# ParBLiSS/kmerhash

Measured on AMD Instinct MI355X. Metric: kmer_inserts_plus_finds_per_sec, higher is better.
Workload: dtype u64

## Files before the change

### kmerhash_amd/csrc/kh_kernels.h

```cpp
#pragma once
#include <hip/hip_runtime.h>
#include <stdint.h>
#include "../../include/kmerhash_amd/kh_hash.h"

#define KH_LB 11
#define KH_L (1u << KH_LB)
#define KH_HS 4096u
#define KH_CHUNK_THREADS 512
#ifndef KH_PART_THREADS
#define KH_PART_THREADS 512
#define KH_PART_MAXPER 4
#endif
#ifndef KH_PART_ITEMS
#define KH_PART_ITEMS 16
#endif
#define KH_PART_TILE (KH_PART_THREADS * KH_PART_ITEMS)
#ifndef KH_PART_STAGE
#define KH_PART_STAGE 4096
#endif
#define KH_NONE 0xFFFFFFFFFFFFFFFFull
#define KH_EMPTY_KEY 0xFFFFFFFFFFFFFFFFull

enum { KHK_RH = 0, KHK_LP = 1 };
enum { KH_FLAG_PROBE_OVERFLOW = 0, KH_FLAG_REGION_OVERFLOW = 1, KH_FLAG_COUNT_OVERFLOW = 2, KH_FLAG_INTERNAL = 3, KH_FLAG_FUSE_INVALID = 4, KH_NFLAGS = 8 };
// ... 406 lines not shown
      for (uint32_t w = 0; w < KH_SCAN_THREADS / 64; ++w) { const uint64_t x = wsum[c][w]; if (w < wid) wpre += x; tot += x; }
      uint64_t ex = running + wpre + incl[c] - ((uint64_t)v[c][0] + v[c][1] + v[c][2] + v[c][3]);
      const uint64_t i0 = base + (uint64_t)c * KH_SCAN_CHUNK + 4 * tid;
#pragma unroll
      for (int j = 0; j < 4; ++j) { if (i0 + j < n) out[i0 + j] = ex; ex += v[c][j]; }
      running += tot;
    }
    __syncthreads();
    if (tid == 0) carry_s = running;
    __syncthreads();
  }
  if (tid == 0) out[n] = carry_s;
}

__global__ __launch_bounds__(256) void k_compact_hits(const uint8_t* __restrict__ flags, const uint64_t* __restrict__ q, const uint32_t* __restrict__ vals,
                               uint64_t n, const uint64_t* __restrict__ tile_off,
                               uint64_t* __restrict__ out_keys, uint32_t* __restrict__ out_vals, uint8_t* __restrict__ out_pairs16) {
  __shared__ uint64_t lk[KH_CMP_TILE];
  __shared__ uint32_t lv[KH_CMP_TILE];
  __shared__ uint32_t wtot[4];
  const uint32_t tid = threadIdx.x, lane = tid & 63, wid = tid >> 6;
  const uint64_t tbase = (uint64_t)blockIdx.x * KH_CMP_TILE;
  const uint64_t base = tbase + (uint64_t)tid * 8;
  uint64_t fw = 0;
  if (base + 8 <= n) fw = *reinterpret_cast<const uint64_t*>(flags + base);
  else for (int j = 0; j < 8; ++j) if (base + j < n && flags[base + j]) fw |= 1ull << (8 * j);
  uint32_t c = 0;
#pragma unroll
  for (int j = 0; j < 8; ++j) c += ((fw >> (8 * j)) & 0xFFu) ? 1u : 0u;
  uint32_t incl = c;
  for (int off = 1; off < 64; off <<= 1) {
    uint32_t o = __shfl_up(incl, off, 64);
    if (lane >= (uint32_t)off) incl += o;
  }
  if (lane == 63) wtot[wid] = incl;
  __syncthreads();
  uint32_t wpre = 0, total = 0;
  for (uint32_t w = 0; w < 4; ++w) { if (w < wid) wpre += wtot[w]; total += wtot[w]; }
  uint32_t x = wpre + incl - c;
#pragma unroll
  for (int j = 0; j < 8; ++j) {
    if ((fw >> (8 * j)) & 0xFFu) { lk[x] = q[base + j]; lv[x] = vals ? vals[base + j] : 0u; ++x; }
  }
  __syncthreads();
  const uint64_t obase = tile_off[blockIdx.x];
  for (uint32_t s = tid; s < total; s += 256) {
    if (out_pairs16) {
      uint4 w;
      w.x = (uint32_t)lk[s]; w.y = (uint32_t)(lk[s] >> 32); w.z = lv[s]; w.w = 0;
      *reinterpret_cast<uint4*>(out_pairs16 + (obase + s) * 16) = w;
    } else {
      out_keys[obase + s] = lk[s];
      if (out_vals) out_vals[obase + s] = lv[s];
    }
  }
}

struct KhTile { uint64_t beg; uint32_t len; uint32_t seg; };
struct KhRec12 { uint32_t klo, khi, val; };

struct KhPartParams {
  const char* kbase; uint32_t kstride;
  const char* vbase; uint32_t vstride;
  uint32_t vconst;
  uint64_t idx_base;
  const ulonglong2* rec_in;
  uint64_t n;
  const KhTile* tiles;
  const uint32_t* ntiles_dev;
  uint32_t ntiles;
  KhSeed seed;
  uint32_t PB;
  uint32_t shift;
  uint32_t nb;
  uint32_t* counts;
  unsigned long long* cursor;
  ulonglong2* orec;
  uint64_t slot;
  uint64_t dump;
  uint32_t* overflow;
  int xcd_swizzle;
  uint64_t slot_in; const unsigned long long* cur_in; uint32_t tps;
  uint64_t sub_slot; uint32_t seg_shift; int xcd_buckets;
};

__device__ __forceinline__ uint32_t kh_part_q(uint64_t h, uint32_t PB) {
  if (PB == 0) return 0;
  uint32_t p = (uint32_t)(h >> KH_LB) & ((1u << PB) - 1u);
  return __brev(p) >> (32 - PB);
}

__device__ __forceinline__ KhTile kh_get_tile(const KhPartParams& P, uint32_t t) {
  if (P.tiles) return P.tiles[t];
  KhTile d;
  d.beg = (uint64_t)t * KH_PART_TILE;
  uint64_t rem = P.n - d.beg;
  d.len = rem < KH_PART_TILE ? (uint32_t)rem : KH_PART_TILE;
  d.seg = 0;
  return d;
}

template <int HASH, bool REC8 = false>
__global__ __launch_bounds__(KH_PART_THREADS) void k_part_hist(KhPartParams P) {
  extern __shared__ __align__(16) uint32_t kh_dyn_smem[];
  uint32_t* hist = kh_dyn_smem;
  const uint32_t tid = threadIdx.x, nb = P.nb;
  const uint32_t ntiles = P.tiles ? *P.ntiles_dev : P.ntiles;
  for (uint32_t i = tid; i < nb; i += KH_PART_THREADS) hist[i] = 0;
  __syncthreads();
  const uint32_t tpb = (ntiles + gridDim.x - 1) / gridDim.x;
  const uint32_t t0 = blockIdx.x * tpb;
  const uint32_t t1 = (t0 + tpb < ntiles) ? t0 + tpb : ntiles;
  uint32_t cur_seg = 0xFFFFFFFFu;
  for (uint32_t t = t0; t < t1; ++t) {
    KhTile d = kh_get_tile(P, t);
    if (d.seg != cur_seg) {
      if (cur_seg != 0xFFFFFFFFu) {
        __syncthreads();
        for (uint32_t i = tid; i < nb; i += KH_PART_THREADS) {
          uint32_t c = hist[i];
          if (c) { atomicAdd(&P.counts[(uint64_t)cur_seg * nb + i], c); hist[i] = 0; }
        }
        __syncthreads();
      }
      cur_seg = d.seg;
    }
    for (uint32_t i = tid; i < d.len; i += KH_PART_THREADS) {
      uint64_t key = P.rec_in ? (REC8 ? reinterpret_cast<const uint64_t*>(P.rec_in)[d.beg + i] : P.rec_in[d.beg + i].x)
                              : *reinterpret_cast<const uint64_t*>(P.kbase + (d.beg + i) * P.kstride);
      uint32_t q = kh_part_q(kh_hash64<HASH>(key, P.seed), P.PB);
      atomicAdd(&hist[(q >> P.shift) & (nb - 1)], 1u);
    }
  }
  __syncthreads();
  if (cur_seg != 0xFFFFFFFFu)
    for (uint32_t i = tid; i < nb; i += KH_PART_THREADS) {
      uint32_t c = hist[i];
      if (c) atomicAdd(&P.counts[(uint64_t)cur_seg * nb + i], c);
    }
}

__device__ __forceinline__ void kh_rec_set(ulonglong2& r, uint64_t key, unsigned long long iv) { r = make_ulonglong2(key, iv); }
__device__ __forceinline__ void kh_rec_set(KhRec12& r, uint64_t key, unsigned long long iv) { r.klo = (uint32_t)key; r.khi = (uint32_t)(key >> 32); r.val = (uint32_t)iv; }
__device__ __forceinline__ void kh_rec_get(const ulonglong2& r, uint64_t& key, unsigned long long& iv) { key = r.x; iv = r.y; }
__device__ __forceinline__ void kh_rec_get(const KhRec12& r, uint64_t& key, unsigned long long& iv) { key = r.klo | ((uint64_t)r.khi << 32); iv = r.val; }
struct KhRec8 { uint64_t key; };
__device__ __forceinline__ void kh_rec_set(KhRec8& r, uint64_t key, unsigned long long) { r.key = key; }
__device__ __forceinline__ void kh_rec_get(const KhRec8& r, uint64_t& key, unsigned long long& iv) { key = r.key; iv = 0; }
template <int RK> struct KhRecOf { typedef ulonglong2 type; };
template <> struct KhRecOf<1> { typedef KhRec12 type; };
template <> struct KhRecOf<2> { typedef KhRec8 type; };
#ifdef KH_PART_OCC3
#define KH_PART_LB(RK) __launch_bounds__(KH_PART_THREADS, (RK) ? 6 : 4)
#define KH_PART_STAGE_OF(RK) ((RK) == 1 ? 3072u : (uint32_t)KH_PART_STAGE)
#else
#define KH_PART_LB(RK) __launch_bounds__(KH_PART_THREADS)
#define KH_PART_STAGE_OF(RK) ((uint32_t)KH_PART_STAGE)
#endif
template <int HASH, int RK>
__global__ KH_PART_LB(RK) void k_part_scatter(KhPartParams P) {
  constexpr bool R12 = RK != 0;
  constexpr uint32_t STAGE = KH_PART_STAGE_OF(RK);
  typedef typename KhRecOf<RK>::type Rec;
  extern __shared__ __align__(16) uint32_t kh_dyn_smem[];
  __shared__ Rec lrec[STAGE];
  __shared__ uint16_t ld[STAGE];
  __shared__ uint32_t wtot[KH_PART_THREADS / 64];
  const uint32_t nb = P.nb;
  uint32_t* hist = kh_dyn_smem;
  uint32_t* loff = kh_dyn_smem + nb;
  unsigned long long* gbase = reinterpret_cast<unsigned long long*>(kh_dyn_smem + 2 * ((nb + 1u) & ~1u));
  const uint32_t tid = threadIdx.x, lane = tid & 63, wid = tid >> 6;
  const uint32_t ntiles = P.tiles ? *P.ntiles_dev : P.ntiles;
  if (blockIdx.x >= ntiles) return;
  uint32_t tile = blockIdx.x;
  const uint32_t xcd = blockIdx.x & 7u;
  if (P.xcd_buckets) {
    const uint32_t j = tile >> 3, per = 8u * P.tps, i = j / per;
    tile = (i * 8u + xcd) * per + (j - i * per);
  } else if (P.xcd_swizzle && (tile | 63u) < ntiles) {
    const uint32_t x = tile & 7u, j = (tile >> 3) & 7u;
    tile = (tile & ~63u) + x * 8u + j;
  }
  KhTile d;
  uint32_t last;
  unsigned long long fill_end = 0;
  if (P.slot_in) {
    const uint32_t seg = tile / P.tps, k = tile - seg * P.tps;
    fill_end = P.cur_in[seg];
    d.seg = seg; d.beg = (uint64_t)seg * P.slot_in + (uint64_t)k * KH_PART_TILE; d.len = 0;
    const uint64_t room = P.slot_in - (uint64_t)k * KH_PART_TILE;
    last = (room < KH_PART_TILE ? (uint32_t)room : KH_PART_TILE) - 1u;
  } else {
    d = kh_get_tile(P, tile);
    if (d.len == 0) return;
    last = d.len - 1u;
  }
  for (uint32_t i = tid; i < nb; i += KH_PART_THREADS) hist[i] = 0;
  uint64_t key[KH_PART_ITEMS];
  unsigned long long iv[KH_PART_ITEMS];
  uint32_t dr[KH_PART_ITEMS];
  if (P.rec_in) {
    const Rec* src = reinterpret_cast<const Rec*>(P.rec_in) + d.beg;
    Rec rr[KH_PART_ITEMS];
#pragma unroll
    for (int j = 0; j < KH_PART_ITEMS; ++j) { const uint32_t i = tid + j * KH_PART_THREADS; rr[j] = src[i < last ? i : last]; }
#pragma unroll
    for (int j = 0; j < KH_PART_ITEMS; ++j) kh_rec_get(rr[j], key[j], iv[j]);
  } else {
    const char* kb = P.kbase + d.beg * P.kstride;
#pragma unroll
    for (int j = 0; j < KH_PART_ITEMS; ++j) {
      const uint32_t i = tid + j * KH_PART_THREADS, ic = i < last ? i : last;
      key[j] = *reinterpret_cast<const uint64_t*>(kb + (uint64_t)ic * P.kstride);
    }
    if (P.vbase) {
      const char* vb = P.vbase + d.beg * P.vstride;
#pragma unroll
      for (int j = 0; j < KH_PART_ITEMS; ++j) {
        const uint32_t i = tid + j * KH_PART_THREADS, ic = i < last ? i : last;
        iv[j] = *reinterpret_cast<const uint32_t*>(vb + (uint64_t)ic * P.vstride);
      }
    } else {
#pragma unroll
      for (int j = 0; j < KH_PART_ITEMS; ++j) iv[j] = P.vconst;
    }
    if (!R12) {
      const uint64_t pos0 = P.idx_base + d.beg;
#pragma unroll
      for (int j = 0; j < KH_PART_ITEMS; ++j) iv[j] |= (unsigned long long)(pos0 + tid + j * KH_PART_THREADS) << 32;
    }
  }
  if (P.slot_in) {
    const uint64_t sbeg = (uint64_t)d.seg * P.slot_in;
    uint64_t fill = fill_end - sbeg;
    if (fill > P.slot_in) fill = P.slot_in;
    const uint64_t off = d.beg - sbeg;
    if (off == (uint64_t)(P.tps - 1u) * KH_PART_TILE && fill > (uint64_t)P.tps * KH_PART_TILE && tid == 0) *P.overflow = 1u;
    d.len = fill > off ? (fill - off < KH_PART_TILE ? (uint32_t)(fill - off) : KH_PART_TILE) : 0u;
    if (d.len == 0) return;
  }
  __syncthreads();
#pragma unroll
  for (int j = 0; j < KH_PART_ITEMS; ++j) {
    const uint32_t i = tid + j * KH_PART_THREADS;
    const uint32_t q = kh_part_q(kh_hash64<HASH>(key[j], P.seed), P.PB);
    const uint32_t dg = (q >> P.shift) & (nb - 1);
    dr[j] = dg << 16;
    if (i < d.len) dr[j] |= atomicAdd(&hist[dg], 1u);
  }
  __syncthreads();
  const uint32_t per = (nb + KH_PART_THREADS - 1) / KH_PART_THREADS;
  uint32_t mine = 0;
  for (uint32_t k = 0; k < per; ++k) { uint32_t b = tid * per + k; if (b < nb) mine += hist[b]; }
  uint32_t incl = mine;
  for (int off = 1; off < 64; off <<= 1) {
    uint32_t o = __shfl_up(incl, off, 64);
// ... 49 lines not shown
      reinterpret_cast<Rec*>(P.orec)[pos] = lrec[s];
    }
  }
}

#define KH_FULLHIST_THREADS 1024
template <int HASH>
__global__ __launch_bounds__(KH_FULLHIST_THREADS) void k_part_hist_full(const char* __restrict__ kbase, uint32_t kstride, uint64_t n, KhSeed seed,
                                                                         uint32_t PB, uint32_t slice, uint32_t slice_bits,
                                                                         uint32_t* __restrict__ counts ) {
  extern __shared__ __align__(16) uint32_t kh_dyn_smem[];
  const uint32_t lb = PB - slice_bits;
  const uint32_t words = lb ? (1u << (lb - 1)) : 1u;
  const uint32_t lmask = (1u << lb) - 1u;
  for (uint32_t i = threadIdx.x; i < words; i += KH_FULLHIST_THREADS) kh_dyn_smem[i] = 0;
  __syncthreads();
  const uint64_t per = (n + gridDim.x - 1) / gridDim.x;
  const uint64_t b0 = (uint64_t)blockIdx.x * per;
  const uint64_t b1 = b0 + per < n ? b0 + per : n;
  for (uint64_t i0 = b0 + threadIdx.x; i0 < b1; i0 += 8 * KH_FULLHIST_THREADS) {
    uint64_t key[8];
#pragma unroll
    for (int j = 0; j < 8; ++j) {
      const uint64_t i = i0 + (uint64_t)j * KH_FULLHIST_THREADS;
      key[j] = i < b1 ? *reinterpret_cast<const uint64_t*>(kbase + i * kstride) : 0ull;
    }
#pragma unroll
    for (int j = 0; j < 8; ++j) {
      if (i0 + (uint64_t)j * KH_FULLHIST_THREADS >= b1) break;
      const uint32_t qg = kh_part_q(kh_hash64<HASH>(key[j], seed), PB);
      if (slice_bits && (qg >> lb) != slice) continue;
      const uint32_t q = qg & lmask;
      const uint32_t sh = 16u * (q & 1u);
      const uint32_t old = atomicAdd(&kh_dyn_smem[q >> 1], 1u << sh);
      if ((((old >> sh) & 0xFFFFu) + 1u) == 0x8000u) {
        atomicSub(&kh_dyn_smem[q >> 1], 0x8000u << sh);
        atomicAdd(&counts[qg], 0x8000u);
      }
    }
  }
  counts += (size_t)slice << lb;
  __syncthreads();
  for (uint32_t i = threadIdx.x; i < words; i += KH_FULLHIST_THREADS) {
    const uint32_t w = kh_dyn_smem[i];
    if (w & 0xFFFFu) atomicAdd(&counts[2 * i], w & 0xFFFFu);
    if (w >> 16) atomicAdd(&counts[2 * i + 1], w >> 16);
  }
}
__global__ void k_seg_offsets(const uint64_t* __restrict__ part_off, uint32_t nb1, uint32_t nb2, uint64_t* __restrict__ segoff,
                              unsigned long long* __restrict__ cur1) {
  const uint32_t s = blockIdx.x * blockDim.x + threadIdx.x;
  if (s <= nb1) { const uint64_t v = part_off[(uint64_t)s * nb2]; segoff[s] = v; if (s < nb1) cur1[s] = v; }
}

__device__ __forceinline__ uint32_t kh_wave_append(bool want, uint32_t* counter);
template <int HASH>
__global__ __launch_bounds__(512) void k_part_direct(const char* __restrict__ kbase, uint32_t kstride, const char* __restrict__ vbase, uint32_t vstride,
                                                     uint32_t vconst, uint64_t n, KhSeed seed, uint32_t PB, ulonglong2* __restrict__ orec,
                                                     unsigned long long* __restrict__ cursor, uint64_t* __restrict__ starts) {
  __shared__ uint32_t cnt;
  const uint32_t q = blockIdx.x, tid = threadIdx.x;
  if (tid == 0) cnt = 0;
  __syncthreads();
  for (uint64_t i0 = 0; i0 < n; i0 += 512) {
    const uint64_t i = i0 + tid;
    bool take = false;
    uint64_t key = 0;
    if (i < n) {
      key = *reinterpret_cast<const uint64_t*>(kbase + i * kstride);
      take = kh_part_q(kh_hash64<HASH>(key, seed), PB) == q;
    }
    const uint32_t pos = kh_wave_append(take, &cnt);
    if (take) {
      const unsigned long long iv = ((unsigned long long)i << 32) | (vbase ? *reinterpret_cast<const uint32_t*>(vbase + i * vstride) : vconst);
      orec[(uint64_t)q * n + pos] = make_ulonglong2(key, iv);
    }
  }
  __syncthreads();
  if (tid == 0) { cursor[q] = (uint64_t)q * n + cnt; starts[q] = (uint64_t)q * n; if (q == 0) starts[gridDim.x] = (uint64_t)gridDim.x * n; }
}

#define KH_SAMPLE_N 65536u
#define KH_SAMPLE_SET (1u << 18)
__global__ void k_sample_dups(const char* __restrict__ kbase, uint32_t kstride, uint64_t n, unsigned long long* __restrict__ set ,
                              uint32_t* __restrict__ dups) {
  const uint32_t i = blockIdx.x * blockDim.x + threadIdx.x;
  if (i >= KH_SAMPLE_N) return;
  const uint64_t pos = (uint64_t)i * (n / KH_SAMPLE_N);
  const unsigned long long key = *reinterpret_cast<const uint64_t*>(kbase + pos * kstride) ^ 0x8000000000000001ull;
  const unsigned long long tag = key ? key : 1ull;
  uint32_t slot = (uint32_t)kh_fmix64(tag) & (KH_SAMPLE_SET - 1);
  for (;;) {
    const unsigned long long cur = atomicCAS(&set[slot], 0ull, tag);
    if (cur == 0ull) break;
    if (cur == tag) { atomicAdd(dups, 1u); break; }
    slot = (slot + 1) & (KH_SAMPLE_SET - 1);
  }
}

__global__ void k_init_cursors2(unsigned long long* __restrict__ cur1, uint64_t n1, uint64_t slot1, uint32_t sub1, unsigned long long* __restrict__ cur2,
                                uint64_t* __restrict__ starts, uint64_t n2, uint64_t slot2, uint32_t* __restrict__ ovf) {
  const uint64_t i = (uint64_t)blockIdx.x * blockDim.x + threadIdx.x;
  if (i < n1 * sub1) cur1[i] = (i / sub1) * slot1 + (i % sub1) * (slot1 / sub1);
  if (i < n2) cur2[i] = i * slot2;
  if (i <= n2) starts[i] = i * slot2;
  if (i == 0) *ovf = 0u;
}
__global__ void k_init_cursors(unsigned long long* __restrict__ cursor, uint64_t* __restrict__ starts, uint64_t n, uint64_t slot) {
  const uint64_t i = (uint64_t)blockIdx.x * blockDim.x + threadIdx.x;
  if (i < n) cursor[i] = i * slot;
  if (starts && i <= n) starts[i] = i * slot;
}

__global__ void k_make_tiles(const uint64_t* __restrict__ segoff, uint32_t nseg, KhTile* __restrict__ tiles, uint32_t* __restrict__ ntiles_out,
                             const unsigned long long* __restrict__ cursor = nullptr, uint64_t slot = 0) {
  __shared__ uint32_t wtot[16];
  __shared__ uint32_t carry_s;
  const uint32_t tid = threadIdx.x, lane = tid & 63, wid = tid >> 6;
  if (tid == 0) carry_s = 0;
  __syncthreads();
  for (uint32_t base = 0; base < nseg; base += 1024) {
    uint32_t s = base + tid;
    uint64_t beg = 0, len = 0;
    if (s < nseg) {
      if (slot) { beg = (uint64_t)s * slot; len = cursor[s] - beg; if (len > slot) len = slot; }
      else { beg = segoff[s]; len = segoff[s + 1] - beg; }
    }
    uint32_t nt = (uint32_t)((len + KH_PART_TILE - 1) / KH_PART_TILE);
    uint32_t incl = nt;
    for (int off = 1; off < 64; off <<= 1) {
      uint32_t o = __shfl_up(incl, off, 64);
      if (lane >= (uint32_t)off) incl += o;
    }
    if (lane == 63) wtot[wid] = incl;
    __syncthreads();
    uint32_t wpre = 0;
    for (uint32_t w = 0; w < wid; ++w) wpre += wtot[w];
    uint32_t carry = carry_s;
    uint32_t first = carry + wpre + incl - nt;
    for (uint32_t k = 0; k < nt; ++k) {
      KhTile d;
      d.beg = beg + (uint64_t)k * KH_PART_TILE;
      uint64_t rem = len - (uint64_t)k * KH_PART_TILE;
      d.len = rem < KH_PART_TILE ? (uint32_t)rem : KH_PART_TILE;
      d.seg = s;
      tiles[first + k] = d;
    }
    __syncthreads();
    if (tid == 1023) carry_s = carry + wpre + incl;
    __syncthreads();
  }
  if (tid == 0) *ntiles_out = carry_s;
}


struct KhMP { long long A; long long n; };
#define KH_MP_NEG (-(1ll << 60))
__device__ __forceinline__ KhMP kh_mp_combine(KhMP first, KhMP then) {
  KhMP r;
  long long a = first.A + then.n;
  r.A = then.A > a ? then.A : a;
  r.n = first.n + then.n;
  return r;
}
__device__ __forceinline__ KhMP kh_block_scan_mp(KhMP v, KhMP* s_wtot, KhMP* total) {
  const uint32_t tid = threadIdx.x, lane = tid & 63, wid = tid >> 6, nw = blockDim.x >> 6;
  KhMP incl = v;
  for (int off = 1; off < 64; off <<= 1) {
    KhMP o;
    o.A = __shfl_up(incl.A, off, 64);
    o.n = __shfl_up(incl.n, off, 64);
    if (lane >= (uint32_t)off) incl = kh_mp_combine(o, incl);
  }
  KhMP excl;
  excl.A = __shfl_up(incl.A, 1, 64);
  excl.n = __shfl_up(incl.n, 1, 64);
  if (lane == 0) { excl.A = KH_MP_NEG; excl.n = 0; }
  __syncthreads();
  if (lane == 63) s_wtot[wid] = incl;
  __syncthreads();
  KhMP wpre; wpre.A = KH_MP_NEG; wpre.n = 0;
  for (uint32_t w = 0; w < wid; ++w) wpre = kh_mp_combine(wpre, s_wtot[w]);
  if (total) {
    KhMP t = wpre;
    for (uint32_t w = wid; w < nw; ++w) t = kh_mp_combine(t, s_wtot[w]);
    *total = t;
  }
  return kh_mp_combine(wpre, excl);
}

// ... 531 lines not shown
      for (uint32_t i = threadIdx.x; i < n; i += KH_CHUNK_THREADS) {
        const uint64_t key = P.ck[b + i];
        f(key, P.cv[b + i], kh_hash64<HASH>(key, P.seed) & mask_n);
      }
    }
  }
}

#define KH_HOMES_PER_THREAD (KH_L / KH_CHUNK_THREADS)

template <int KIND, int HASH>
__global__ __launch_bounds__(KH_CHUNK_THREADS) void k_chunk_count(KhRebuildParams P) {
  __shared__ uint32_t cnt[KH_L];
  __shared__ uint32_t s_emin;
  __shared__ KhMP s_wtot[KH_CHUNK_THREADS / 64];
  const uint32_t tid = threadIdx.x, c = blockIdx.x;
  const uint32_t Ln = P.New.cap > KH_L ? KH_L : (uint32_t)P.New.cap;
  const uint64_t Sc = (uint64_t)c * Ln;
  for (uint32_t i = tid; i < KH_L; i += KH_CHUNK_THREADS) cnt[i] = 0;
  __syncthreads();
  kh_for_each_old<KIND, HASH>(P, c, &s_emin, [&](uint64_t, uint32_t, uint64_t hn) { atomicAdd(&cnt[hn - Sc], 1u); });
  kh_for_each_new<HASH>(P, c, [&](uint64_t, uint32_t, uint64_t hn) { atomicAdd(&cnt[hn - Sc], 1u); });
  __syncthreads();
  KhMP v; v.A = KH_MP_NEG; v.n = 0;
#pragma unroll
  for (uint32_t j = 0; j < KH_HOMES_PER_THREAD; ++j) {
    uint32_t b = tid * KH_HOMES_PER_THREAD + j;
    if (b < Ln) {
      uint32_t cb = cnt[b];
      if (cb > 0xFFFFu) { atomicOr(&P.flags[KH_FLAG_COUNT_OVERFLOW], 1u); cb = 0xFFFFu; }
      P.homecnt[Sc + b] = (uint16_t)cb;
      KhMP h; h.A = (long long)b + cb; h.n = cb;
      v = kh_mp_combine(v, h);
    }
  }
  KhMP total;
  kh_block_scan_mp(v, s_wtot, &total);
  if (tid == 0) { P.sumA[c] = (long long)Sc + total.A; P.sumN[c] = total.n; }
}

#define KH_CARRY_ITEMS 8
__global__ void k_chunk_carry(const long long* __restrict__ sumA, const long long* __restrict__ sumN, uint32_t nch, long long cap,
                              long long* __restrict__ xcarry, KhMP* __restrict__ prefix_tmp) {
  __shared__ KhMP s_wtot[16];
  __shared__ KhMP s_carry;
  const uint32_t tid = threadIdx.x;
  if (tid == 0) { s_carry.A = KH_MP_NEG; s_carry.n = 0; }
  __syncthreads();
  for (uint32_t base = 0; base < nch; base += 1024 * KH_CARRY_ITEMS) {
    const uint32_t c0 = base + tid * KH_CARRY_ITEMS;
    KhMP it[KH_CARRY_ITEMS];
    KhMP v; v.A = KH_MP_NEG; v.n = 0;
#pragma unroll
    for (int j = 0; j < KH_CARRY_ITEMS; ++j) {
      it[j].A = KH_MP_NEG; it[j].n = 0;
      if (c0 + j < nch) { it[j].A = sumA[c0 + j]; it[j].n = sumN[c0 + j]; }
      v = kh_mp_combine(v, it[j]);
    }
    KhMP total;
    KhMP excl = kh_block_scan_mp(v, s_wtot, &total);
    const KhMP carry = s_carry;
    KhMP run = kh_mp_combine(carry, excl);
#pragma unroll
    for (int j = 0; j < KH_CARRY_ITEMS; ++j) {
      if (c0 + j < nch) prefix_tmp[c0 + j] = run;
      run = kh_mp_combine(run, it[j]);
    }
    __syncthreads();
    if (tid == 0) s_carry = kh_mp_combine(carry, total);
    __syncthreads();
  }
  KhMP all = s_carry;
  long long end0 = all.A > all.n ? all.A : all.n;
  long long x0 = end0 - cap;
  if (x0 < 0) x0 = 0;
  for (uint32_t c = tid; c < nch; c += 1024) {
    KhMP p = prefix_tmp[c];
    long long x = x0 + p.n;
    xcarry[c] = p.A > x ? p.A : x;
  }
}

#define KH_SPILL 256
template <int KIND, int HASH>
__global__ __launch_bounds__(KH_CHUNK_THREADS) void k_chunk_place(KhRebuildParams P) {
  __shared__ uint64_t skeys[KH_L + KH_SPILL];
  __shared__ uint32_t svals[KH_L + KH_SPILL];
  __shared__ uint32_t sinfo_w[(KH_L + KH_SPILL) / 4];
  __shared__ uint32_t fill[KH_L];
  __shared__ uint32_t start[KH_L];
  __shared__ uint32_t s_emin;
  __shared__ long long s_pend;
  __shared__ KhMP s_wtot[KH_CHUNK_THREADS / 64];
  uint8_t* sinfo = reinterpret_cast<uint8_t*>(sinfo_w);
  const uint32_t tid = threadIdx.x, c = blockIdx.x;
  const uint32_t Ln = P.New.cap > KH_L ? KH_L : (uint32_t)P.New.cap;
  const uint64_t Sc = (uint64_t)c * Ln, mask_n = P.New.cap - 1;
  const uint32_t empty4 = KIND == KHK_RH ? 0u : 0x40404040u;
  for (uint32_t i = tid; i < KH_L + KH_SPILL; i += KH_CHUNK_THREADS) { skeys[i] = 0; svals[i] = 0; }
  for (uint32_t i = tid; i < (KH_L + KH_SPILL) / 4; i += KH_CHUNK_THREADS) sinfo_w[i] = empty4;
  uint32_t cb[KH_HOMES_PER_THREAD];
  KhMP v; v.A = KH_MP_NEG; v.n = 0;
#pragma unroll
  for (uint32_t j = 0; j < KH_HOMES_PER_THREAD; ++j) {
    uint32_t b = tid * KH_HOMES_PER_THREAD + j;
    cb[j] = b < Ln ? P.homecnt[Sc + b] : 0u;
    if (b < Ln) { KhMP h; h.A = (long long)b + cb[j]; h.n = cb[j]; v = kh_mp_combine(v, h); }
    fill[tid * KH_HOMES_PER_THREAD + j] = 0;
  }
  KhMP excl = kh_block_scan_mp(v, s_wtot, nullptr);
  const long long xr = P.xcarry[c] - (long long)Sc;
  long long p = excl.A > xr + excl.n ? excl.A : xr + excl.n;
#pragma unroll
  for (uint32_t j = 0; j < KH_HOMES_PER_THREAD; ++j) {
    uint32_t b = tid * KH_HOMES_PER_THREAD + j;
    if (b < Ln) {
      long long st = p > (long long)b ? p : (long long)b;
      start[b] = (uint32_t)st;
      p = st + cb[j];
    }
  }
  if (tid == KH_CHUNK_THREADS - 1) s_pend = p;
  __syncthreads();
  auto place = [&](uint64_t key, uint32_t val, uint64_t hn) {
    uint32_t b = (uint32_t)(hn - Sc);
    uint32_t r = atomicAdd(&fill[b], 1u);
    uint32_t prel = start[b] + r;
    uint32_t dist = prel - b;
    uint8_t ib = 0x00;
    if (KIND == KHK_RH) {
      if (dist > 127u) { atomicOr(&P.flags[KH_FLAG_PROBE_OVERFLOW], 1u); dist = 127u; }
      ib = (uint8_t)(0x80u | dist);
    }
    if (prel < KH_L + KH_SPILL) { skeys[prel] = key; svals[prel] = val; sinfo[prel] = ib; }
    else kh_slot_st(P.New.s + ((Sc + prel) & mask_n), key, val, ib);
  };
  kh_for_each_old<KIND, HASH>(P, c, &s_emin, place);
  kh_for_each_new<HASH>(P, c, place);
  __syncthreads();
  long long pend = s_pend;
  if (pend < (long long)Ln) pend = Ln;
  const uint32_t lo = xr > 0 ? (uint32_t)xr : 0u;
  uint32_t hi = pend < (long long)(KH_L + KH_SPILL) ? (uint32_t)pend : (KH_L + KH_SPILL);
  for (uint32_t s0 = lo + tid; s0 < hi; s0 += KH_CHUNK_THREADS) {
    kh_slot_st(P.New.s + ((Sc + s0) & mask_n), skeys[s0], svals[s0], sinfo[s0]);
  }
}

#define KH_XB 127u
#define KH_FSPILL 128u
struct KhFusedParams {
  KhSrcSet src; uint32_t PB;
  KhSlots New; KhSeed seed; int mode;
  unsigned long long* pub;
  uint64_t* ck0; uint32_t* cv0; uint16_t* homecnt0;
  uint32_t* maxidx;
  uint64_t n_total, half_max_load;
  uint64_t base_size;
  unsigned long long* est;
  uint32_t* flags;
  long long poll_limit;
  int nodup;
  KhRebuildParams R;
};

template <int KIND, int HASH, bool MERGE>
__device__ __forceinline__ uint32_t kh_stage_from_table(const KhRebuildParams& R, uint32_t c, uint64_t Sc, unsigned long long* lk,
                                                         unsigned long long* liv, uint32_t* n_staged, uint32_t* scratch) {
  const uint32_t tid = threadIdx.x;
  const uint64_t cap_o = R.Old.cap, mask_o = cap_o - 1, mask_n = R.New.cap - 1;
  if (tid == 0) *n_staged = 0;
  __syncthreads();
  if (cap_o) {
    const uint32_t nch_o = (uint32_t)(cap_o >> KH_LB);
    const uint32_t o = c & (nch_o - 1);
    const bool same = R.New.cap == cap_o;
    const uint64_t S = (uint64_t)o * KH_L;
    uint64_t len = KH_L + 128u;
    if (KIND == KHK_LP) {
      const uint64_t beyond = cap_o - KH_L;
      uint64_t e_total = beyond;
      for (uint64_t base = 0; base < beyond; base += KH_L) {
        const uint32_t window = beyond - base < KH_L ? (uint32_t)(beyond - base) : KH_L;
        __syncthreads();
        if (tid == 0) *scratch = window;
        __syncthreads();
        for (uint32_t t = tid; t < window; t += KH_CHUNK_THREADS) {
          if ((R.Old.s[(S + KH_L + base + t) & mask_o].info & 0xFFu) == 0x40u) { atomicMin(scratch, t); break; }
        }
        __syncthreads();
        const uint32_t e = *scratch;
        e_total = base + e;
        if (e < window) break;
      }
      __syncthreads();
      if (tid == 0) *scratch = 0;
      len = KH_L + e_total;
    }
    if (KIND == KHK_RH) {
      constexpr uint32_t NS = (KH_L + 128u + KH_CHUNK_THREADS - 1) / KH_CHUNK_THREADS;
      uint4 w[NS];
#pragma unroll
      for (uint32_t it = 0; it < NS; ++it) {
        const uint32_t t = it * KH_CHUNK_THREADS + tid;
        w[it] = kh_slot_ld(R.Old.s + ((S + (t < KH_L + 128u ? t : KH_L + 127u)) & mask_o));
      }
#pragma unroll
      for (uint32_t it = 0; it < NS; ++it) {
        const uint64_t sl = (S + it * KH_CHUNK_THREADS + tid) & mask_o;
        const uint32_t inf = it * KH_CHUNK_THREADS + tid < KH_L + 128u ? (w[it].w & 0xFFu) : 0u;
        bool take = false;
        uint32_t hrel = 0;
        const uint64_t key = kh_slot_key(w[it]);
        if (inf >= 0x80u && !(R.drop_marked && (w[it].w & KH_INFO_ERASE_MARK))) {
          const uint64_t home_o = (sl - (inf & 0x7Fu)) & mask_o;
          if ((uint32_t)(home_o >> KH_LB) == o) {
            if (same) { take = true; hrel = (uint32_t)(home_o - S); }
            else {
              const uint64_t hn = kh_hash64<HASH>(key, R.seed) & mask_n;
              take = (uint32_t)(hn >> KH_LB) == c;
              hrel = (uint32_t)(hn - Sc);
            }
          }
        }
        const uint32_t x = kh_wave_append(take, n_staged);
        if (take && x < KH_DD_M) { lk[x] = key; liv[x] = MERGE ? (unsigned long long)w[it].z : (((unsigned long long)hrel << 32) | w[it].z); }
      }
    } else
    for (uint64_t t0 = 0; t0 < len; t0 += KH_CHUNK_THREADS) {
      const uint64_t t = t0 + tid;
      bool take = false;
      uint64_t key = 0; uint32_t val = 0, hrel = 0;
      if (t < len) {
        const uint4 w = kh_slot_ld(R.Old.s + ((S + t) & mask_o));
        if ((w.w & 0xFFu) < 0x40u) {
          key = kh_slot_key(w);
          const uint64_t h = kh_hash64<HASH>(key, R.seed);
          if ((uint32_t)((h & mask_o) >> KH_LB) == o && (uint32_t)((h & mask_n) >> KH_LB) == c) {
            take = true; val = w.z; hrel = (uint32_t)((h & mask_n) - Sc);
          }
        }
      }
      const uint32_t x = kh_wave_append(take, n_staged);
      if (take && x < KH_DD_M) { lk[x] = key; liv[x] = MERGE ? (unsigned long long)val : (((unsigned long long)hrel << 32) | val); }
    }
  }
  if (!MERGE)
    kh_for_each_new<HASH>(R, c, [&](uint64_t key, uint32_t val, uint64_t hn) {
      const uint32_t x = kh_wave_append(true, n_staged);
      if (x < KH_DD_M) { lk[x] = key; liv[x] = ((unsigned long long)(uint32_t)(hn - Sc) << 32) | val; }
    });
  __syncthreads();
  return *n_staged;
}

#ifdef KH_TRACE
__device__ unsigned long long kh_trace[512 * 12];
#ifndef KH_TRACE_SRC
#define KH_TRACE_SRC 0
#endif
#define KH_STAMP(i) do { if (SRC == KH_TRACE_SRC && threadIdx.x == 0 && blockIdx.x >= 20000 && blockIdx.x < 20512) kh_trace[(blockIdx.x - 20000) * 12 + (i)] = clock64(); } while (0)
#else
#define KH_STAMP(i)
#endif
template <int KIND, int HASH, int SRC>
__global__ __launch_bounds__(KH_CHUNK_THREADS) void k_build_fused(KhFusedParams P) {
  __shared__ unsigned long long lk[KH_DD_M];
  __shared__ unsigned long long liv[KH_DD_M];
  __shared__ uint32_t set[KH_HS];
  __shared__ __align__(8) uint16_t simg[KH_L + KH_FSPILL];
  __shared__ KhMP32 s_wtot[KH_CHUNK_THREADS / 64];
  __shared__ uint32_t s_chunk, s_x, s_max, s_abort;
  __shared__ long long s_pend;
  static_assert(KH_HS >= 2 * KH_L, "set[] is reused as cnt/fill + start");
  uint32_t* cnt = set;
  uint32_t* start = set + KH_L;
  const uint32_t tid = threadIdx.x;
  const uint64_t cap = P.New.cap, mask_n = cap - 1;
  const uint32_t nch = (uint32_t)(cap >> KH_LB);
  KH_STAMP(0);
  if (tid == 0) {
    s_chunk = blockIdx.x;
    s_max = 0;
    s_abort = (SRC == 0 || SRC == 2) ? (uint32_t)__hip_atomic_load(&P.est[1], __ATOMIC_RELAXED, __HIP_MEMORY_SCOPE_AGENT) : 0u;
  }
  __syncthreads();
  const ulonglong2** s_ptr = reinterpret_cast<const ulonglong2**>(simg);
  uint32_t* s_cum = reinterpret_cast<uint32_t*>(simg) + 2 * KH_MAX_SRC;
  static_assert((KH_L + KH_FSPILL) * 2 >= KH_MAX_SRC * 8 + (KH_MAX_SRC + 1) * 4, "source table fits the image array");
  const uint32_t c = s_chunk;
  const uint64_t Sc = (uint64_t)c * KH_L;
  const unsigned long long VALID = 1ull << 63;
  uint32_t m, rep_mask;
  uint32_t vote_old = 0, vote_rec = 0;
  if (SRC == 0) {
    const uint32_t q = P.PB ? (__brev(c) >> (32 - P.PB)) : 0u;
    const KhSrcView V = kh_src_setup<true>(P.src, q, s_ptr, s_cum);
    m = V.m;
    KH_STAMP(1);
    vote_rec = m;
    const bool aborted = s_abort != 0;
    if (m >= KH_DD_M || aborted) {
      if (tid == 0) {
        if (!aborted) atomicOr(&P.flags[KH_FLAG_FUSE_INVALID], 1u);
        __hip_atomic_store(&P.pub[c], VALID, __ATOMIC_RELAXED, __HIP_MEMORY_SCOPE_AGENT);
      }
      return;
    }
    const bool nodup = P.nodup && c != 0;
    if (!nodup) for (uint32_t s = tid; s < KH_HS; s += KH_CHUNK_THREADS) set[s] = 0;
    if (m) {
      ulonglong2 rr[KH_DD_M / KH_CHUNK_THREADS];
      const uint32_t last = m - 1u;
      if (V.one12) {
        KhRec12 r3[KH_DD_M / KH_CHUNK_THREADS];
#pragma unroll
        for (uint32_t it = 0; it < KH_DD_M / KH_CHUNK_THREADS; ++it) { const uint32_t i = it * KH_CHUNK_THREADS + tid; r3[it] = V.one12[i < last ? i : last]; }
#pragma unroll
        for (uint32_t it = 0; it < KH_DD_M / KH_CHUNK_THREADS; ++it) rr[it] = make_ulonglong2(r3[it].klo | ((uint64_t)r3[it].khi << 32), (unsigned long long)r3[it].val);
      } else if (V.one) {
#pragma unroll
        for (uint32_t it = 0; it < KH_DD_M / KH_CHUNK_THREADS; ++it) { const uint32_t i = it * KH_CHUNK_THREADS + tid; rr[it] = V.one[i < last ? i : last]; }
      } else {
        const ulonglong2* pp[KH_DD_M / KH_CHUNK_THREADS];
#pragma unroll
        for (uint32_t it = 0; it < KH_DD_M / KH_CHUNK_THREADS; ++it) { const uint32_t i = it * KH_CHUNK_THREADS + tid; pp[it] = kh_src_addr(V, s_ptr, s_cum, i < last ? i : last); }
#pragma unroll
        for (uint32_t it = 0; it < KH_DD_M / KH_CHUNK_THREADS; ++it) rr[it] = *pp[it];
      }
#pragma unroll
      for (uint32_t it = 0; it < KH_DD_M / KH_CHUNK_THREADS; ++it) {
        const uint32_t i = it * KH_CHUNK_THREADS + tid;
        if (i < m) { lk[i] = rr[it].x; liv[i] = rr[it].y; }
      }
    }
    if (V.n > 1) __syncthreads();
    for (uint32_t i = tid; i < KH_L + KH_FSPILL; i += KH_CHUNK_THREADS) simg[i] = 0xFFFFu;
    __syncthreads();
    if (nodup) {
      rep_mask = 0;
#pragma unroll
      for (uint32_t it = 0; it < KH_DD_M / KH_CHUNK_THREADS; ++it) if (it * KH_CHUNK_THREADS + tid < m) rep_mask |= 1u << it;
    } else rep_mask = kh_dd_fold(lk, liv, set, m, P.mode, P.seed.xk);
    __syncthreads();
    KH_STAMP(2);
  } else if (SRC == 2) {
    const uint32_t q = P.PB ? (__brev(c) >> (32 - P.PB)) : 0u;
    const KhSrcView V = kh_src_setup(P.src, q, s_ptr, s_cum);
    for (uint32_t s = tid; s < KH_HS; s += KH_CHUNK_THREADS) set[s] = 0;
    if (s_abort != 0) {
      if (tid == 0) __hip_atomic_store(&P.pub[c], VALID, __ATOMIC_RELAXED, __HIP_MEMORY_SCOPE_AGENT);
      return;
    }
    const uint32_t n_old = kh_stage_from_table<KIND, HASH, true>(P.R, c, Sc, lk, liv, &s_x, &s_max);
    KH_STAMP(1);
    m = n_old + V.m;
    vote_old = n_old; vote_rec = V.m;
    if (n_old >= KH_DD_M || m >= KH_DD_M) {
      if (tid == 0) {
        atomicOr(&P.flags[KH_FLAG_FUSE_INVALID], 1u);
        __hip_atomic_store(&P.pub[c], VALID, __ATOMIC_RELAXED, __HIP_MEMORY_SCOPE_AGENT);
      }
      return;
// ... 234 lines not shown
    constexpr uint32_t KH_DUPK = 3;
    uint32_t ei[KH_DD_M / KH_CHUNK_THREADS][KH_DUPK];
#pragma unroll
    for (uint32_t it = 0; it < KH_DD_M / KH_CHUNK_THREADS; ++it)
#pragma unroll
      for (uint32_t d = 0; d < KH_DUPK; ++d) ei[it][d] = simg[pr[it] + d < gend[it] ? pr[it] + d : 0u] & 0x7FFu;
    bool more = false;
#pragma unroll
    for (uint32_t it = 0; it < KH_DD_M / KH_CHUNK_THREADS; ++it) {
#pragma unroll
      for (uint32_t d = 0; d < KH_DUPK; ++d)
        if (kh_keq(lk[ei[it][d]], mykey[it], P.seed.xk) && pr[it] + d < gend[it]) dup = true;
      pr[it] += KH_DUPK;
      more = more || pr[it] < gend[it];
    }
    while (__any(more)) {
      more = false;
#pragma unroll
      for (uint32_t it = 0; it < KH_DD_M / KH_CHUNK_THREADS; ++it) {
        if (pr[it] < gend[it]) {
          if (kh_keq(lk[simg[pr[it]] & 0x7FFu], mykey[it], P.seed.xk)) dup = true;
          ++pr[it];
          more = more || pr[it] < gend[it];
        }
      }
    }
    if (__any(dup) && (tid & 63) == 0) atomicOr(&P.flags[KH_FLAG_FUSE_INVALID], 1u);
  }
  KH_STAMP(7);
  long long pend = s_pend;
  if (pend < (long long)KH_L) pend = KH_L;
  const uint32_t lo = (uint32_t)xr;
  const uint32_t hi = pend < (long long)(KH_L + KH_FSPILL) ? (uint32_t)pend : (KH_L + KH_FSPILL);
  for (uint32_t s0 = lo + tid; s0 < hi; s0 += KH_CHUNK_THREADS) {
    KhSlot* dst = P.New.s + ((Sc + s0) & mask_n);
    const uint32_t e = simg[s0];
    if (e == 0xFFFFu) kh_slot_st(dst, 0, 0, kh_empty_info<KIND>());
    else {
      const uint32_t x = e & 0x7FFu;
      const uint64_t key = lk[x];
      uint32_t ib = 0x00u;
      if (KIND == KHK_RH) {
        uint32_t dist = e >> 11;
        if (dist == 31u) {
          dist = s0 - (uint32_t)((kh_hash64<HASH>(key, P.seed) & mask_n) - Sc);
          if (dist > 127u) dist = 127u;
        }
        ib = 0x80u | dist;
      }
      kh_slot_st(dst, key, (uint32_t)liv[x], ib);
    }
  }
  KH_STAMP(8);
}

#ifdef KH_TRACE
#define KH_STAMP_L(i) do { if (threadIdx.x == 0 && blockIdx.x >= 20000 && blockIdx.x < 20512) kh_trace[(blockIdx.x - 20000) * 12 + (i)] = clock64(); } while (0)
#else
#define KH_STAMP_L(i)
#endif
#define KH_LEAN_M 2016u
template <int KIND, int HASH>
__global__ __launch_bounds__(KH_CHUNK_THREADS, 8) void k_build_lean(KhFusedParams P) {
  __shared__ unsigned long long lk[KH_LEAN_M];
  __shared__ uint32_t lv[KH_LEAN_M];
  __shared__ __align__(16) uint32_t cnt16[KH_L / 2];
  __shared__ __align__(8) uint16_t start0[KH_L];
  __shared__ __align__(16) uint16_t u_sort[KH_L + KH_LEAN_M];
  uint16_t* npre = u_sort;
  uint16_t* sidx = u_sort + KH_L;
  uint16_t* simg = u_sort;
  static_assert(KH_L + KH_LEAN_M >= KH_L + KH_FSPILL, "the slot image fits over the sort arrays");
  static_assert(((KH_L + KH_FSPILL) * 2) % 16 == 0 && (KH_L * 2) % 16 == 0, "filled with 16-byte stores");
  __shared__ KhMP32 s_wtot[KH_CHUNK_THREADS / 64];
  __shared__ uint32_t s_x, s_abort;
  __shared__ long long s_pend;
  const uint32_t tid = threadIdx.x;
  const uint64_t cap = P.New.cap, mask_n = cap - 1;
  const uint32_t nch = (uint32_t)(cap >> KH_LB);
  const uint32_t c = blockIdx.x;
  const uint64_t Sc = (uint64_t)c * KH_L;
  const unsigned long long VALID = 1ull << 63;
  KH_STAMP_L(0);
  if (tid == 0) s_abort = (uint32_t)__hip_atomic_load(&P.est[1], __ATOMIC_RELAXED, __HIP_MEMORY_SCOPE_AGENT);
  const uint32_t q = P.PB ? (__brev(c) >> (32 - P.PB)) : 0u;
  const KhRec12* src; uint32_t m;
  KhRec12 r3[KH_DD_M / KH_CHUNK_THREADS];
  unsigned long long kreg[KH_DD_M / KH_CHUNK_THREADS];
  if (P.src.slot[0]) {
    const uint64_t b = (uint64_t)q * P.src.slot[0];
    src = reinterpret_cast<const KhRec12*>(P.src.rec[0]) + b;
    const uint32_t last = (uint32_t)P.src.slot[0] - 1u;
#pragma unroll
    for (uint32_t it = 0; it < KH_DD_M / KH_CHUNK_THREADS; ++it) { const uint32_t i = it * KH_CHUNK_THREADS + tid; r3[it] = src[i < last ? i : last]; }
    const uint64_t e = P.src.cur[0][q] - b;
    m = (uint32_t)(e < P.src.slot[0] ? e : P.src.slot[0]);
  } else {
    const uint64_t b = P.src.off[0][q];
    src = reinterpret_cast<const KhRec12*>(P.src.rec[0]) + b;
    m = (uint32_t)(P.src.off[0][q + 1] - b);
    const uint32_t last = m ? m - 1u : 0u;
    const KhRec12* from = m ? src : reinterpret_cast<const KhRec12*>(P.src.rec[0]);
#pragma unroll
    for (uint32_t it = 0; it < KH_DD_M / KH_CHUNK_THREADS; ++it) { const uint32_t i = it * KH_CHUNK_THREADS + tid; r3[it] = from[i < last ? i : last]; }
  }
  kh_lds_fill16(cnt16, sizeof(cnt16), 0u);
  __syncthreads();
  const bool aborted = s_abort != 0;
  if (m >= KH_LEAN_M || aborted) {
    if (tid == 0) {
      if (!aborted) atomicOr(&P.flags[KH_FLAG_FUSE_INVALID], 1u);
      __hip_atomic_store(&P.pub[c], VALID, __ATOMIC_RELAXED, __HIP_MEMORY_SCOPE_AGENT);
    }
    return;
  }
  uint32_t hb[KH_DD_M / KH_CHUNK_THREADS];
#pragma unroll
  for (uint32_t it = 0; it < KH_DD_M / KH_CHUNK_THREADS; ++it) {
    const uint32_t i = it * KH_CHUNK_THREADS + tid;
    kreg[it] = r3[it].klo | ((uint64_t)r3[it].khi << 32);
    hb[it] = 0;
    if (i < m) {
      lk[i] = kreg[it]; lv[i] = r3[it].val;
      hb[it] = (uint32_t)((kh_hash64<HASH>(kreg[it], P.seed) & mask_n) - Sc) & (KH_L - 1u);
      atomicAdd(&cnt16[hb[it] >> 1], 1u << (16 * (hb[it] & 1)));
    }
  }
  KH_STAMP_L(1);
  __syncthreads();
  KH_STAMP_L(2);
  uint32_t cb[KH_HOMES_PER_THREAD];
  KhMP32 v; v.A = KH_MP32_NEG; v.n = 0;
#pragma unroll
  for (uint32_t j = 0; j < KH_HOMES_PER_THREAD; ++j) {
    const uint32_t b = tid * KH_HOMES_PER_THREAD + j;
    cb[j] = (cnt16[b >> 1] >> (16 * (b & 1))) & 0xFFFFu;
    KhMP32 h; h.A = (int)(b + cb[j]); h.n = (int)cb[j];
    v = kh_mp_combine(v, h);
  }
  KhMP32 total;
  const KhMP32 excl = kh_block_scan_mp32(v, s_wtot, &total);
  const uint32_t n_c = (uint32_t)total.n;
  const long long spill0 = total.A > (long long)KH_L ? total.A - (long long)KH_L : 0;
  const bool early = n_c + KH_XB <= KH_L;
  KH_STAMP_L(3);
  if (c == 0) {
    bool dup = false;
#pragma unroll
    for (uint32_t it = 0; it < KH_DD_M / KH_CHUNK_THREADS; ++it) {
      const uint32_t x = it * KH_CHUNK_THREADS + tid;
      if (x < m) {
        for (uint32_t y = x + 1; y < m; ++y) dup = dup || kh_keq(lk[y], kreg[it], P.seed.xk);
      }
    }
    if (__any(dup) && (tid & 63) == 0) atomicOr(&P.flags[KH_FLAG_FUSE_INVALID], 1u);
    if (tid == 0) {
      if (!early) atomicOr(&P.flags[KH_FLAG_FUSE_INVALID], 1u);
      __hip_atomic_store(&P.pub[0], VALID | ((unsigned long long)spill0 << 32) | n_c, __ATOMIC_RELAXED, __HIP_MEMORY_SCOPE_AGENT);
      P.maxidx[0] = 0;
    }
#pragma unroll
    for (uint32_t j = 0; j < KH_HOMES_PER_THREAD; ++j) P.homecnt0[tid * KH_HOMES_PER_THREAD + j] = (uint16_t)cb[j];
    for (uint32_t x = tid; x < m; x += KH_CHUNK_THREADS) { P.ck0[x] = lk[x]; P.cv0[x] = lv[x]; }
    return;
  }
  unsigned long long w0 = 0;
  if (tid == 0) {
    if (c < 64) {
      const unsigned long long mine = ((unsigned long long)n_c << 32) | m;
      const unsigned long long tot = atomicAdd(&P.est[0], mine) + mine;
      const uint32_t sn = (uint32_t)(tot >> 32), sm = (uint32_t)tot;
      if ((c == 63 || (nch < 64 && c == nch - 1)) && sm > 0) {
        const double dhat = (double)P.base_size + (double)P.n_total * (double)sn / (double)sm * 1.15;
        if (dhat <= (double)P.half_max_load) {
          atomicOr(&P.flags[KH_FLAG_FUSE_INVALID], 1u);
          __hip_atomic_store(&P.est[1], 1ull, __ATOMIC_RELAXED, __HIP_MEMORY_SCOPE_AGENT);
        }
      }
    }
    if (early) __hip_atomic_store(&P.pub[c], VALID | ((unsigned long long)spill0 << 32) | n_c, __ATOMIC_RELAXED, __HIP_MEMORY_SCOPE_AGENT);
    w0 = __hip_atomic_load(&P.pub[c - 1], __ATOMIC_RELAXED, __HIP_MEMORY_SCOPE_AGENT);
    P.maxidx[c] = 0;
  }
  {
    long long p = excl.A > (long long)excl.n ? excl.A : excl.n;
    uint32_t np = (uint32_t)excl.n;
    uint32_t st4[KH_HOMES_PER_THREAD], np4[KH_HOMES_PER_THREAD];
#pragma unroll
    for (uint32_t j = 0; j < KH_HOMES_PER_THREAD; ++j) {
      const uint32_t b = tid * KH_HOMES_PER_THREAD + j;
      const long long st = p > (long long)b ? p : (long long)b;
      st4[j] = (uint32_t)st & 0xFFFFu;
      np4[j] = np;
      p = st + cb[j];
      np += cb[j];
    }
    static_assert(KH_HOMES_PER_THREAD == 4, "two packed counter words, one 8-byte store of starts / counts per thread");
    reinterpret_cast<uint2*>(start0)[tid] = make_uint2(st4[0] | (st4[1] << 16), st4[2] | (st4[3] << 16));
    reinterpret_cast<uint2*>(npre)[tid] = make_uint2(np4[0] | (np4[1] << 16), np4[2] | (np4[3] << 16));
    if (tid == KH_CHUNK_THREADS - 1) s_pend = p;
    cnt16[tid * (KH_HOMES_PER_THREAD / 2)] = 0; cnt16[tid * (KH_HOMES_PER_THREAD / 2) + 1] = 0;
  }
  __syncthreads();
  uint32_t pj[KH_DD_M / KH_CHUNK_THREADS];
#pragma unroll
  for (uint32_t it = 0; it < KH_DD_M / KH_CHUNK_THREADS; ++it) {
    pj[it] = 0;
    const uint32_t x = it * KH_CHUNK_THREADS + tid;
    if (x < m) {
      const uint32_t b = hb[it];
      const uint32_t r = (atomicAdd(&cnt16[b >> 1], 1u << (16 * (b & 1))) >> (16 * (b & 1))) & 0xFFFFu;
      uint32_t j = npre[b] + r;
      if (j >= KH_LEAN_M) j = KH_LEAN_M - 1u;
      sidx[j] = (uint16_t)x;
      pj[it] = (start0[b] + r) | (j << 16);
    }
  }
  __syncthreads();
  KH_STAMP_L(4);
  {
    bool dup = false;
    uint32_t jn[KH_DD_M / KH_CHUNK_THREADS], gend[KH_DD_M / KH_CHUNK_THREADS];
#pragma unroll
    for (uint32_t it = 0; it < KH_DD_M / KH_CHUNK_THREADS; ++it) {
      gend[it] = 0;
      const uint32_t x = it * KH_CHUNK_THREADS + tid;
      if (x < m) {
        const uint32_t b = hb[it];
        gend[it] = npre[b] + ((cnt16[b >> 1] >> (16 * (b & 1))) & 0xFFFFu);
        if (gend[it] > KH_LEAN_M) gend[it] = KH_LEAN_M;
      }
      jn[it] = (pj[it] >> 16) + 1u;
    }
    constexpr uint32_t KH_DUPK = 3;
    uint32_t ei[KH_DD_M / KH_CHUNK_THREADS][KH_DUPK];
#pragma unroll
    for (uint32_t it = 0; it < KH_DD_M / KH_CHUNK_THREADS; ++it)
#pragma unroll
      for (uint32_t d = 0; d < KH_DUPK; ++d) ei[it][d] = sidx[jn[it] + d < gend[it] ? jn[it] + d : 0u];
    bool more = false;
#pragma unroll
    for (uint32_t it = 0; it < KH_DD_M / KH_CHUNK_THREADS; ++it) {
#pragma unroll
      for (uint32_t d = 0; d < KH_DUPK; ++d)
        if (kh_keq(lk[ei[it][d] < KH_LEAN_M ? ei[it][d] : 0u], kreg[it], P.seed.xk) && jn[it] + d < gend[it]) dup = true;
      jn[it] += KH_DUPK;
      more = more || jn[it] < gend[it];
    }
    while (__any(more)) {
      more = false;
#pragma unroll
      for (uint32_t it = 0; it < KH_DD_M / KH_CHUNK_THREADS; ++it) {
        if (jn[it] < gend[it]) {
          const uint32_t e = sidx[jn[it]];
          if (kh_keq(lk[e < KH_LEAN_M ? e : 0u], kreg[it], P.seed.xk)) dup = true;
          ++jn[it];
          more = more || jn[it] < gend[it];
        }
      }
    }
    if (__any(dup) && (tid & 63) == 0) atomicOr(&P.flags[KH_FLAG_FUSE_INVALID], 1u);
  }
  KH_STAMP_L(5);
  if (tid == 0) {
    unsigned long long w = w0;
// ... 502 lines not shown
    uint32_t dist = pos - b;
    if (dist > 127u) { atomicOr(&P.flags[KH_FLAG_PROBE_OVERFLOW], 1u); dist = 127u; }
    if (pos < KH_L + KH_FSPILL) { ikey[pos] = key; ival[pos] = val; iinfo[pos] = (uint8_t)(0x80u | dist); }
    else kh_slot_st(P.New.s + ((Sc + pos) & mask_n), key, val, 0x80u | dist);
  };
  uint32_t late = 0;
  uint32_t pj[ROWS + 2];
#pragma unroll
  for (uint32_t k = 0; k < ROWS; ++k) {
    pj[k] = 0;
    if ((keep >> k) & 1u) {
      const uint32_t b = rank[k] >> 16, r = rank[k] & 0xFFFFu;
      const uint32_t p0 = start0[b] + r, j = npre[b] + r;
      pj[k] = (p0 & 0xFFFFu) | (j << 16);
      if (p0 >= KH_XB + j) enter(kh_slot_key(w[k]), w[k].z, b, p0); else late |= 1u << k;
    }
  }
#pragma unroll
  for (uint32_t u = 0; u < 2; ++u) {
    pj[ROWS + u] = 0;
    if (rrank[u] != 0xFFFFFFFFu) {
      const uint32_t i = tid + u * KH_CHUNK_THREADS;
      const uint32_t b = hbr[u], r = rrank[u];
      const uint32_t p0 = start0[b] + r, j = npre[b] + r;
      pj[ROWS + u] = (p0 & 0xFFFFu) | (j << 16);
      if (p0 >= KH_XB + j) enter(rk[i], (uint32_t)riv[i], b, p0); else late |= 1u << (ROWS + u);
    }
  }
  if (tid == 0) {
    unsigned long long ww = w0;
    const long long t0 = clock64();
    while (!(ww & VALID)) {
      if (clock64() - t0 > P.poll_limit) { atomicOr(&P.flags[KH_FLAG_FUSE_INVALID], 1u); ww = VALID; break; }
      __builtin_amdgcn_s_sleep(4);
      ww = __hip_atomic_load(&P.pub[c - 1], __ATOMIC_RELAXED, __HIP_MEMORY_SCOPE_AGENT);
    }
    const uint32_t x = (uint32_t)((ww >> 32) & 0x7FFFFFFFu);
    if (x > KH_XB) atomicOr(&P.flags[KH_FLAG_FUSE_INVALID], 1u);
    if (!early) {
      const long long e = (long long)x + n_c;
      const long long pe = (long long)total.A > e ? (long long)total.A : e;
      const long long sp = pe > (long long)KH_L ? pe - (long long)KH_L : 0;
      __hip_atomic_store(&P.pub[c], VALID | ((unsigned long long)sp << 32) | n_c, __ATOMIC_RELAXED, __HIP_MEMORY_SCOPE_AGENT);
    }
    s_x = x > KH_XB ? 0u : x;
  }
  __syncthreads();
  const uint32_t xr = s_x;
#pragma unroll
  for (uint32_t k = 0; k < ROWS; ++k) {
    if ((late >> k) & 1u) {
      const uint32_t p0 = pj[k] & 0xFFFFu, pc = (pj[k] >> 16) + xr;
      enter(kh_slot_key(w[k]), w[k].z, rank[k] >> 16, p0 > pc ? p0 : pc);
    }
  }
#pragma unroll
  for (uint32_t u = 0; u < 2; ++u) {
    if ((late >> (ROWS + u)) & 1u) {
      const uint32_t i = tid + u * KH_CHUNK_THREADS;
      const uint32_t p0 = pj[ROWS + u] & 0xFFFFu, pc = (pj[ROWS + u] >> 16) + xr;
      enter(rk[i], (uint32_t)riv[i], hbr[u], p0 > pc ? p0 : pc);
    }
  }
  __syncthreads();
  {
    const int tA = total.A > 0 ? total.A : 0;
    int pend = tA > (int)xr + (int)n_c ? tA : (int)xr + (int)n_c;
    if (pend < (int)KH_L) pend = (int)KH_L;
    if (pend > (int)(KH_L + KH_FSPILL)) pend = (int)(KH_L + KH_FSPILL);
#pragma unroll
    for (uint32_t k = 0; k < ROWS; ++k) {
      const int s0 = (int)(base + 64u * k);
      if (k < nrows && s0 >= (int)xr && s0 < pend) {
        const uint32_t ib = iinfo[s0];
        KhSlot* dst = P.New.s + ((Sc + (uint32_t)s0) & mask_n);
        if (ib == 0u) kh_slot_st(dst, 0, 0, kh_empty_info<KHK_RH>());
        else kh_slot_st(dst, ikey[s0], ival[s0], ib);
      }
    }
  }
  (void)n_old;
}

__global__ void k_fused_tail_carry(const unsigned long long* __restrict__ pub, uint32_t nch, long long* __restrict__ xcarry0,
                                   uint64_t* __restrict__ noff0 = nullptr, uint32_t* __restrict__ ncnt0 = nullptr) {
  if (threadIdx.x == 0 && blockIdx.x == 0) {
    xcarry0[0] = (long long)((pub[nch - 1] >> 32) & 0x7FFFFFFFull);
    if (noff0) { noff0[0] = 0; noff0[1] = 0; }
    if (ncnt0) ncnt0[0] = (uint32_t)pub[0];
  }
}

__global__ __launch_bounds__(1024) void k_fused_totals(const unsigned long long* __restrict__ pub, const uint32_t* __restrict__ maxidx, uint32_t nch,
                                                       unsigned long long* __restrict__ totals) {
  __shared__ unsigned long long ws[16];
  __shared__ uint32_t wm[16];
  unsigned long long sum = 0; uint32_t mx = 0;
  for (uint32_t c = blockIdx.x * 1024 + threadIdx.x; c < nch; c += gridDim.x * 1024) { sum += pub[c] & 0xFFFFFFFFull; const uint32_t v = maxidx[c]; mx = v > mx ? v : mx; }
  for (int off = 32; off > 0; off >>= 1) { sum += __shfl_down(sum, off, 64); const uint32_t o = __shfl_down(mx, off, 64); mx = o > mx ? o : mx; }
  if ((threadIdx.x & 63) == 0) { ws[threadIdx.x >> 6] = sum; wm[threadIdx.x >> 6] = mx; }
  __syncthreads();
  if (threadIdx.x == 0) {
    unsigned long long t = 0; uint32_t m = 0;
    for (int w = 0; w < 16; ++w) { t += ws[w]; m = wm[w] > m ? wm[w] : m; }
    if (t) atomicAdd(&totals[0], t);
    if (m) atomicMax(&totals[1], (unsigned long long)m);
  }
}

__global__ void k_disp_hist(const KhSlot* __restrict__ slots, uint64_t cap, unsigned long long* __restrict__ out128) {
  __shared__ uint32_t h[128];
  if (threadIdx.x < 128) h[threadIdx.x] = 0;
  __syncthreads();
  uint64_t i = (uint64_t)blockIdx.x * blockDim.x + threadIdx.x;
  uint64_t stride = (uint64_t)gridDim.x * blockDim.x;
  for (; i < cap; i += stride) { uint32_t b = slots[i].info & 0xFFu; if (b >= 0x80u) atomicAdd(&h[b & 0x7Fu], 1u); }
  __syncthreads();
  if (threadIdx.x < 128 && h[threadIdx.x]) atomicAdd(&out128[threadIdx.x], (unsigned long long)h[threadIdx.x]);
}

template <int KIND>
__global__ void k_unpack_slots(const KhSlot* __restrict__ slots, uint64_t cap, uint64_t* __restrict__ keys, uint32_t* __restrict__ vals,
                               uint8_t* __restrict__ info, uint8_t* __restrict__ flags) {
  uint64_t i = (uint64_t)blockIdx.x * blockDim.x + threadIdx.x;
  uint64_t stride = (uint64_t)gridDim.x * blockDim.x;
  for (; i < cap; i += stride) {
    const uint4 w = kh_slot_ld(slots + i);
    if (keys) keys[i] = kh_slot_key(w);
    if (vals) vals[i] = w.z;
    if (info) info[i] = (uint8_t)(w.w & 0xFFu);
    if (flags) flags[i] = kh_is_occupied<KIND>(w.w & 0xFFu) ? 1 : 0;
  }
}

#define KH_SHARD_THREADS 512
#define KH_SHARD_TILE(KW) (KH_SHARD_THREADS * KhKey<KW>::SHARD_ITEMS)
#define KH_SHARD_MAXR 64
struct KhShardAdj { long long a[8]; __host__ __device__ KhShardAdj() { for (int i = 0; i < 8; ++i) a[i] = 0; } };
__global__ void k_shard_piece_bounds(const uint64_t* __restrict__ tile_off, uint32_t ntiles, uint32_t p, uint32_t pieces, uint64_t* __restrict__ out ) {
  const uint32_t j = blockIdx.x * blockDim.x + threadIdx.x;
  if (j >= p * (pieces + 1)) return;
  const uint32_t r = j / (pieces + 1), i = j % (pieces + 1);
  out[j] = tile_off[(uint64_t)r * ntiles + (uint64_t)ntiles * i / pieces];
}
template <int HASH, int KW>
__device__ __forceinline__ uint32_t kh_rank_of(typename KhKey<KW>::key_t key, typename KhKey<KW>::seed_t seed, uint32_t p, uint32_t pmask) {
  const uint64_t h = KhKey<KW>::template hash<HASH>(key, seed);
  return pmask ? (uint32_t)(h & pmask) : (uint32_t)(h % p);
}
template <int HASH, int KW>
__global__ __launch_bounds__(KH_SHARD_THREADS) void k_shard_count(const uint64_t* __restrict__ keys, uint64_t n, typename KhKey<KW>::seed_t seed, uint32_t p,
                                                                  uint32_t pmask, uint32_t* __restrict__ tile_counts , uint32_t ntiles) {
  typedef KhKey<KW> K;
  __shared__ uint32_t h[KH_SHARD_MAXR];
  if (threadIdx.x < KH_SHARD_MAXR) h[threadIdx.x] = 0;
  __syncthreads();
  const uint64_t base = (uint64_t)blockIdx.x * KH_SHARD_TILE(KW);
  typename K::key_t key[K::SHARD_ITEMS];
#pragma unroll
  for (uint32_t k = 0; k < K::SHARD_ITEMS; ++k) {
    const uint64_t i = base + threadIdx.x + k * KH_SHARD_THREADS;
    key[k] = K::load(keys, i < n ? i : n - 1);
  }
  if (p <= 8) {
    unsigned long long c0 = 0, c1 = 0;
#pragma unroll
    for (uint32_t k = 0; k < K::SHARD_ITEMS; ++k) {
      const uint64_t i = base + threadIdx.x + k * KH_SHARD_THREADS;
      if (i < n) {
        const uint32_t r = kh_rank_of<HASH, KW>(key[k], seed, p, pmask);
        if (r < 4) c0 += 1ull << (16 * r); else c1 += 1ull << (16 * (r - 4));
      }
    }
// ... 640 lines not shown
```

### kmerhash_amd/csrc/kmerhash_amd.hip

```cpp
#include "kh_kernels.h"
#include "kh_kernels_wide.h"
#include "kh_kernels_values.h"
#include "kh_kernels_index.h"
#include "kh_kernels_index_wide.h"
#include "kh_kernels_csr.h"
#include "kh_kernels_chain.h"
#include "kh_kernels_edits.h"
#include "kh_kernels_cigar.h"
#include "kh_kernels_ends.h"
#include "kh_part_sizing.h"
#include "kh_scratch.h"
#include "../../include/kmerhash_amd.h"

#include <string>
#include <vector>
#include <cstdio>
#include <cstring>
#include <algorithm>
#include <cmath>
#include <cstdlib>

#include <map>
#include <memory>
#include <mutex>
// ... 44 lines not shown
    e = hipMalloc(&p, bytes);
    if (e != hipSuccess) return e;
  }
  std::lock_guard<std::mutex> g(P.m);
  P.size_of[p] = bytes;
  *out = p;
  return hipSuccess;
}
void pool_free(int dev, void* p) {
  if (!p) return;
  DevPool& P = g_pool[dev & 15];
  {
    std::lock_guard<std::mutex> g(P.m);
    auto it = P.size_of.find(p);
    if (it != P.size_of.end()) {
      P.free_.insert(std::make_pair(it->second, p));
      P.cached += it->second;
      return;
    }
  }
  hipFree(p);
}
struct HostPool { std::mutex m; std::vector<uint64_t*> pinned; std::vector<hipEvent_t> events[16]; };
HostPool g_host;
uint64_t* pinned_get() {
  { std::lock_guard<std::mutex> g(g_host.m);
    if (!g_host.pinned.empty()) { uint64_t* p = g_host.pinned.back(); g_host.pinned.pop_back(); return p; } }
  uint64_t* p = nullptr;
  if (hipHostMalloc(reinterpret_cast<void**>(&p), 64 * sizeof(uint64_t)) != hipSuccess) { (void)hipGetLastError(); return nullptr; }
  return p;
}
void pinned_put(uint64_t* p) { if (p) { std::lock_guard<std::mutex> g(g_host.m); g_host.pinned.push_back(p); } }
hipEvent_t event_get(int dev) {
  { std::lock_guard<std::mutex> g(g_host.m);
    auto& v = g_host.events[dev & 15];
    if (!v.empty()) { hipEvent_t e = v.back(); v.pop_back(); return e; } }
  hipEvent_t e = nullptr;
  hipEventCreate(&e);
  return e;
}
void event_put(int dev, hipEvent_t e) { if (e) { std::lock_guard<std::mutex> g(g_host.m); g_host.events[dev & 15].push_back(e); } }
}

namespace {

struct ProfRec { const char* name; hipEvent_t a, b; };

struct Block { char* p; size_t cap; };

}

struct SlackShared { unsigned long long* cur2; uint64_t* starts; uint32_t* ovf; uint64_t slot; };
struct SlotBuf {
  void* p; uint64_t cap;
  SlotBuf() : p(nullptr), cap(0) {}
  SlotBuf(KhSlots s) : p(s.s), cap(s.cap) {}
  SlotBuf(KwSlots s) : p(s.s), cap(s.cap) {}
};
struct kh_table {
  int kind = KHK_RH, hash = 0, device = 0;
  KhSeed seed = KhSeed{0, 0u};
  hipStream_t stream = nullptr;
  float min_lf = 0.f, max_lf = 0.f;
  uint64_t min_load = 0, max_load = 0, lsize = 0;
  uint32_t slot_bytes = sizeof(KhSlot);
  SlotBuf cur, spare;
  std::vector<Block> blocks;
  size_t blk = 0, off = 0;
  uint64_t* hpin = nullptr;
  std::string err;
  struct {
    bool active, fallback, nodup; int mode;
    bool repeatable, slack, rec12;
    SlackShared sh;
    uint64_t n_total, fed, cap_u; uint32_t PB;
    ulonglong2 *tmp, *fin;
    KhSrcSet S;
    uint64_t* stage_k; uint32_t* stage_v;
    const uint64_t* wk[KH_MAX_SRC]; const uint32_t* wv[KH_MAX_SRC]; uint64_t wn[KH_MAX_SRC]; uint32_t wsrc; uint32_t* wcnt;
  } ins = {};
  uint32_t* part_overflow = nullptr;
  double batch_vf = 1.0;
  bool batch_nodup = false;
  bool prof = false;
  std::vector<ProfRec> recs;
  std::vector<std::pair<std::string, std::pair<double, uint64_t> > > prof_acc;
};
struct kh_wtable : kh_table {};

namespace {

inline uint64_t next_pow2(uint64_t x) {
  if (x <= 1) return 1;
  return uint64_t(1) << (64 - __builtin_clzll(x - 1));
}
inline uint64_t threshold(uint64_t buckets, float lf) {
  return static_cast<uint64_t>(static_cast<float>(buckets) * lf);
}
inline uint32_t log2u(uint64_t x) { return 63u - (uint32_t)__builtin_clzll(x); }

kh_status fail(kh_table* t, kh_status s, const std::string& msg) {
  if (t) t->err = msg;
  return s;
}
inline kh_status hip_status(hipError_t e) { return e == hipSuccess ? KH_OK : e == hipErrorOutOfMemory ? KH_ERR_NOMEM : KH_ERR_HIP; }
kh_status hip_fail(kh_table* t, const char* call, hipError_t e) {
  if (t) t->err = std::string(call) + ": " + hipGetErrorString(e);
  return hip_status(e);
}
#define HIPCHK_T(table, call)                                                                          \
  do {                                                                                                 \
    hipError_t e__ = (call);                                                                           \
    if (e__ != hipSuccess) return hip_fail(table, #call, e__);                                         \
  } while (0)
#define HIPCHK(call) HIPCHK_T(t, call)
#define HIPCHK0(call) HIPCHK_T(nullptr, call)

inline int cu_count(int device) {
  int ncu = 256;
  hipDeviceGetAttribute(&ncu, hipDeviceAttributeMultiprocessorCount, device);
  return ncu > 0 ? ncu : 256;
}
inline int cu_count(const kh_table* t) { return cu_count(t->device); }

class Scratch {
 public:
  Scratch(int device, hipStream_t stream) : device_(device), stream_(stream) {}
  Scratch(const Scratch&) = delete;
  Scratch& operator=(const Scratch&) = delete;
  ~Scratch() { finish(); }

  hipError_t error() const { return err_; }
  bool ok() const { return err_ == hipSuccess; }
  void check(hipError_t e) { if (err_ == hipSuccess) err_ = e; }
  bool launched() { check(hipGetLastError()); busy_ = true; return ok(); }

  void* alloc(size_t bytes) {
    void* p = nullptr;
    if (ok() && nblk_ == kMaxBlocks) err_ = hipErrorInvalidValue;
    if (ok()) err_ = pool_alloc(device_, bytes, &p);
    if (!ok()) return nullptr;
    blk_[nblk_++] = p;
    busy_ = true;
    return p;
  }
  template <typename F> size_t measure(F&& layout) { car_ = KhCarver(); layout(*this); return car_.size(); }
  template <typename F> void carve(void* base, F&& layout) { car_ = KhCarver(base); layout(*this); }
  template <typename F> bool layout(F&& layout) {
    const size_t bytes = measure(layout);
    void* p = bytes ? alloc(bytes) : nullptr;
    if (bytes && !p) return false;
    carve(p, layout);
    return ok();
  }
  template <typename T> T* take(uint64_t count) { return car_.take<T>(count); }
  template <typename T> const T* in(const T* p, uint64_t count, kh_mem where) {
    if (where != KH_MEM_HOST) return p;
    T* d = car_.take<T>(count);
    if (d) copy(d, p, count * sizeof(T), hipMemcpyHostToDevice);
    return d;
  }
  template <typename T> T* out(T* p, uint64_t count, kh_mem where) {
    if (where != KH_MEM_HOST) return p;
    T* d = car_.take<T>(count);
    if (d && nout_ == kMaxOut) check(hipErrorInvalidValue);
    else if (d) outs_[nout_++] = Out{p, d};
// ... 135 lines not shown
    if (st != KH_OK) return st;
  }
  s = Slots{static_cast<decltype(s.s)>(b.p), cap};
  if (g_poison) {
    if (is_wide(t)) hipLaunchKernelGGL(kw_poison, slots_grid(cap), dim3(256), 0, t->stream, wide(b));
    else hipLaunchKernelGGL(k_poison, slots_grid(cap), dim3(256), 0, t->stream, narrow(b));
    HIPCHK(hipGetLastError());
  }
  return KH_OK;
}
void retire_slots(kh_table* t, SlotBuf s) {
  if (!s.p) return;
  if (t->spare.p) { hipStreamSynchronize(t->stream); free_slots(t, t->spare); }
  t->spare = s;
}
void adopt_slots(kh_table* t, SlotBuf nw) {
  const SlotBuf old = t->cur;
  t->cur = nw;
  retire_slots(t, old);
  t->min_load = threshold(nw.cap, t->min_lf);
  t->max_load = threshold(nw.cap, t->max_lf);
}

struct Launch {
  kh_table* t; const char* name; hipEvent_t a, b; bool on;
  Launch(kh_table* t_, const char* n) : t(t_), name(n), a(nullptr), b(nullptr), on(t_ && t_->prof) {
    if (on) { a = event_get(t->device); b = event_get(t->device); hipEventRecord(a, t->stream); }
  }
  ~Launch() {
    if (on) { hipEventRecord(b, t->stream); ProfRec r; r.name = name; r.a = a; r.b = b; t->recs.push_back(r); }
  }
};
void prof_collect(kh_table* t) {
  if (t->recs.empty()) return;
  hipStreamSynchronize(t->stream);
  for (auto& r : t->recs) {
    float ms = 0.f;
    hipEventElapsedTime(&ms, r.a, r.b);
    event_put(t->device, r.a); event_put(t->device, r.b);
    bool found = false;
    for (auto& a : t->prof_acc) if (a.first == r.name) { a.second.first += ms; a.second.second += 1; found = true; break; }
    if (!found) t->prof_acc.push_back(std::make_pair(std::string(r.name), std::make_pair(double(ms), uint64_t(1))));
  }
  t->recs.clear();
}

#define KH_SWITCH_HASH(h, ...)                                                        \
  switch (h) {                                                                        \
    case KHH_IDENTITY: { constexpr int HASH = KHH_IDENTITY; __VA_ARGS__; } break;     \
    case KHH_MURMUR3_X86: { constexpr int HASH = KHH_MURMUR3_X86; __VA_ARGS__; } break; \
    case KHH_MURMUR3_X64: { constexpr int HASH = KHH_MURMUR3_X64; __VA_ARGS__; } break; \
    default: { constexpr int HASH = KHH_FARM; __VA_ARGS__; } break;                   \
  }
#define KH_SWITCH_KIND_HASH(k, h, ...)                                                \
  if ((k) == KHK_RH) { constexpr int KIND = KHK_RH; KH_SWITCH_HASH(h, __VA_ARGS__) }  \
  else { constexpr int KIND = KHK_LP; KH_SWITCH_HASH(h, __VA_ARGS__) }

inline uint32_t grid_for(uint64_t n, uint32_t block, uint32_t maxblocks = 256 * 16) {
  uint64_t g = (n + block - 1) / block;
  if (g < 1) g = 1;
  if (g > maxblocks) g = maxblocks;
  return (uint32_t)g;
}

template <typename T>
kh_status stage_in(kh_table* t, const void* p, uint64_t n, kh_mem where, const T** out) {
  if (where == KH_MEM_DEVICE || p == nullptr) { *out = static_cast<const T*>(p); return KH_OK; }
  T* d = nullptr;
  TAKE(d, T, n);
  HIPCHK(hipMemcpyAsync(d, p, sizeof(T) * n, hipMemcpyHostToDevice, t->stream));
  *out = d;
  return KH_OK;
}

inline size_t ws_rebuild(uint64_t cap) { return size_t(cap) * 2 + (cap > KH_L ? (cap >> KH_LB) : 1) * 48 + (size_t(1) << 16); }

struct PreCount { uint16_t* homecnt; long long* sumA; long long* sumN; };

const bool g_disable_fused_rebuild = getenv("KH_DISABLE_FUSED_BUILD") != nullptr || getenv("KH_DISABLE_FUSED_REBUILD") != nullptr;

const long long g_poll_limit = getenv("KH_DEBUG_POLL_LIMIT") ? atoll(getenv("KH_DEBUG_POLL_LIMIT")) : (1ll << 23);
struct FusedRun { unsigned long long* totals; uint32_t* flags; };
const bool g_disable_lean = getenv("KH_DISABLE_LEAN_BUILD") != nullptr;
kh_status launch_fused(kh_table* t, int src, KhFusedParams& F, const KhSlots& nw, uint32_t PB_tail, const char* name, FusedRun* out) {
  const uint32_t nch = (uint32_t)(nw.cap >> KH_LB);
  char* blk; uint32_t* maxidx; uint64_t* ck0; uint32_t* cv0; uint16_t* hc0; long long* xc0; uint64_t* noff0; uint32_t* ncnt0;
  const size_t sz_pub = (size_t)nch * 8, sz_ctl = sz_pub + 256, sz_all = sz_ctl + (size_t)nch * 4;
  TAKE(blk, char, sz_all);
  maxidx = reinterpret_cast<uint32_t*>(blk + sz_ctl);
  TAKE(ck0, uint64_t, KH_DD_M); TAKE(cv0, uint32_t, KH_DD_M); TAKE(hc0, uint16_t, KH_L); TAKE(xc0, long long, 1);
  TAKE(noff0, uint64_t, 2); TAKE(ncnt0, uint32_t, 1);
  HIPCHK(hipMemsetAsync(blk, 0, sz_all, t->stream));
  F.New = nw; F.seed = t->seed;
  F.pub = reinterpret_cast<unsigned long long*>(blk);
  unsigned long long* totals = reinterpret_cast<unsigned long long*>(blk + sz_pub);
  F.maxidx = maxidx; F.ck0 = ck0; F.cv0 = cv0; F.homecnt0 = hc0;
  F.est = reinterpret_cast<unsigned long long*>(blk + sz_pub + 32);
  F.flags = reinterpret_cast<uint32_t*>(blk + sz_pub + 64);
  F.poll_limit = g_poll_limit;
  F.R.New = nw; F.R.seed = t->seed; F.R.flags = F.flags;
  { Launch L(t, name);
    const double mean_c = (double)F.n_total / (double)nch;
    const bool lean_fits = mean_c + 5.0 * std::sqrt(mean_c) < (double)KH_LEAN_M;
    if (src == 0 && F.nodup && F.src.rec12 == 1 && F.src.n == 1 && lean_fits && !g_disable_lean) { KH_SWITCH_KIND_HASH(t->kind, t->hash, hipLaunchKernelGGL((k_build_lean<KIND, HASH>), dim3(nch), dim3(KH_CHUNK_THREADS), 0, t->stream, F)); }
    else if (src == 0) { KH_SWITCH_KIND_HASH(t->kind, t->hash, hipLaunchKernelGGL((k_build_fused<KIND, HASH, 0>), dim3(nch), dim3(KH_CHUNK_THREADS), 0, t->stream, F)); }
    else if (src == 1) { KH_SWITCH_KIND_HASH(t->kind, t->hash, hipLaunchKernelGGL((k_build_fused<KIND, HASH, 1>), dim3(nch), dim3(KH_CHUNK_THREADS), 0, t->stream, F)); }
    else if (src == 3) { KH_SWITCH_HASH(t->hash, hipLaunchKernelGGL((k_build_fused<KHK_RH, HASH, 3>), dim3(nch), dim3(KH_CHUNK_THREADS), 0, t->stream, F)); }
    else if (src == 4) { KH_SWITCH_HASH(t->hash, hipLaunchKernelGGL((k_erase_stream<HASH>), dim3(nch), dim3(KH_CHUNK_THREADS), 0, t->stream, F)); }
    else if (src == 5) { KH_SWITCH_HASH(t->hash, hipLaunchKernelGGL((k_insert_stream<HASH>), dim3(nch), dim3(KH_CHUNK_THREADS), 0, t->stream, F)); }
    else { KH_SWITCH_KIND_HASH(t->kind, t->hash, hipLaunchKernelGGL((k_build_fused<KIND, HASH, 2>), dim3(nch), dim3(KH_CHUNK_THREADS), 0, t->stream, F)); } }
  { Launch L(t, "k_fused_totals");
    hipLaunchKernelGGL(k_fused_totals, dim3(std::max<uint32_t>(1u, std::min<uint32_t>(64u, nch / 1024u))), dim3(1024), 0, t->stream, F.pub, maxidx, nch, totals); }
  {
    Launch L(t, "k_fused_tail");
    hipLaunchKernelGGL(k_fused_tail_carry, dim3(1), dim3(64), 0, t->stream, F.pub, nch, xc0, noff0, ncnt0);
    KhRebuildParams T0;
    memset(&T0, 0, sizeof(T0));
    T0.Old = kNoSlots; T0.New = nw; T0.ck = ck0; T0.cv = cv0; T0.noff = noff0; T0.ncnt = ncnt0; T0.PB = PB_tail;
    T0.seed = t->seed; T0.homecnt = hc0; T0.xcarry = xc0; T0.flags = F.flags;
    KH_SWITCH_KIND_HASH(t->kind, t->hash, hipLaunchKernelGGL((k_chunk_place<KIND, HASH>), dim3(1), dim3(KH_CHUNK_THREADS), 0, t->stream, T0));
  }
  HIPCHK(hipGetLastError());
  HIPCHK(hipMemcpyAsync(t->hpin, blk + sz_pub, 128, hipMemcpyDeviceToHost, t->stream));
  t->hpin[30] = 0;
  if (t->part_overflow) HIPCHK(hipMemcpyAsync(t->hpin + 30, t->part_overflow, 4, hipMemcpyDeviceToHost, t->stream));
  HIPCHK(hipStreamSynchronize(t->stream));
  out->totals = totals; out->flags = F.flags;
  return KH_OK;
}

const char* const kProbeOverflowText = "Robin Hood probe distance would exceed 127 (7-bit info field, hashmap_robinhood.hpp:142-144,556)";
const char* const kDedupOverflowText = "internal: de-duplication set overflow";
kh_status flags_status(kh_table* t, const uint32_t* f) {
  if (f[KH_FLAG_PROBE_OVERFLOW]) return fail(t, KH_ERR_PROBE_OVERFLOW, kProbeOverflowText);
  if (f[KH_FLAG_REGION_OVERFLOW]) return fail(t, KH_ERR_PROBE_OVERFLOW, "cluster longer than one chunk (2048 slots) without an empty slot");
  if (f[KH_FLAG_COUNT_OVERFLOW]) return fail(t, KH_ERR_PROBE_OVERFLOW, "more than 65535 keys share one home bucket");
  if (f[KH_FLAG_INTERNAL]) return fail(t, KH_ERR_HIP, kDedupOverflowText);
  return KH_OK;
}

struct Narrow {
  typedef KhSlots Slots; typedef KhRebuildParams Params;
  static Slots view(const SlotBuf& b) { return narrow(b); }
  static void set_seed(Params& P, const kh_table* t) { P.seed = t->seed; }
  static void count(kh_table* t, uint32_t nch, const Params& P) {
    Launch L(t, "k_chunk_count");
    KH_SWITCH_KIND_HASH(t->kind, t->hash, hipLaunchKernelGGL((k_chunk_count<KIND, HASH>), dim3(nch), dim3(KH_CHUNK_THREADS), 0, t->stream, P));
  }
  static void place(kh_table* t, uint32_t nch, const Params& P) {
    Launch L(t, "k_chunk_place");
    KH_SWITCH_KIND_HASH(t->kind, t->hash, hipLaunchKernelGGL((k_chunk_place<KIND, HASH>), dim3(nch), dim3(KH_CHUNK_THREADS), 0, t->stream, P));
  }
};
struct Wide {
  typedef KwSlots Slots; typedef KwRebuildParams Params;
  static Slots view(const SlotBuf& b) { return wide(b); }
  static void set_seed(Params& P, const kh_table* t) { P.seed = t->seed.s; }
  static void count(kh_table* t, uint32_t nch, const Params& P) {
    Launch L(t, "kw_chunk_count");
    KH_SWITCH_HASH(t->hash, hipLaunchKernelGGL((kw_chunk_count<HASH>), dim3(nch), dim3(KW_DD_THREADS), 0, t->stream, P));
  }
  static void place(kh_table* t, uint32_t nch, const Params& P) {
    Launch L(t, "kw_chunk_place");
    KH_SWITCH_HASH(t->hash, hipLaunchKernelGGL((kw_chunk_place<HASH>), dim3(nch), dim3(KW_DD_THREADS), 0, t->stream, P));
  }
};
template <typename W>
kh_status relayout(kh_table* t, typename W::Slots nw, const uint64_t* ck, const uint32_t* cv, const uint64_t* noff, const uint32_t* ncnt,
                   uint32_t PB, bool drop_marked, const PreCount* pre) {
  const uint32_t nch = nw.cap > KH_L ? (uint32_t)(nw.cap >> KH_LB) : 1u;
  uint16_t* homecnt; long long *sumA, *sumN, *xcarry; KhMP* ptmp; uint32_t* flags;
  if (pre) { homecnt = pre->homecnt; sumA = pre->sumA; sumN = pre->sumN; }
  else { TAKE(homecnt, uint16_t, nw.cap); TAKE(sumA, long long, nch); TAKE(sumN, long long, nch); }
  TAKE(xcarry, long long, nch);
  TAKE(ptmp, KhMP, nch);
  TAKE(flags, uint32_t, KH_NFLAGS);
  HIPCHK(hipMemsetAsync(flags, 0, sizeof(uint32_t) * KH_NFLAGS, t->stream));
  typename W::Params P;
  memset(&P, 0, sizeof(P));
  P.Old = W::view(t->cur); P.drop_marked = drop_marked ? 1 : 0; P.New = nw; P.ck = ck; P.cv = cv; P.noff = noff; P.ncnt = ncnt; P.PB = PB;
  if (t->lsize == 0) P.Old.cap = 0;
  W::set_seed(P, t); P.homecnt = homecnt; P.sumA = sumA; P.sumN = sumN; P.xcarry = xcarry; P.flags = flags;
  if (!pre) W::count(t, nch, P);
  { Launch L(t, "k_chunk_carry");
    hipLaunchKernelGGL(k_chunk_carry, dim3(1), dim3(1024), 0, t->stream, sumA, sumN, nch, (long long)nw.cap, xcarry, ptmp); }
  W::place(t, nch, P);
  HIPCHK(hipGetLastError());
  HIPCHK(hipMemcpyAsync(t->hpin, flags, sizeof(uint32_t) * KH_NFLAGS, hipMemcpyDeviceToHost, t->stream));
  HIPCHK(hipStreamSynchronize(t->stream));
  const kh_status st = flags_status(t, reinterpret_cast<const uint32_t*>(t->hpin));
  if (st != KH_OK) { retire_slots(t, nw); return st; }
  adopt_slots(t, nw);
  return KH_OK;
}

kh_status rebuild(kh_table* t, uint64_t new_cap, const uint64_t* ck, const uint32_t* cv, const uint64_t* noff,
                  const uint32_t* ncnt, uint32_t PB, bool drop_marked, uint64_t total_after, const PreCount* pre = nullptr) {
  if (total_after > new_cap)
    return fail(t, KH_ERR_FULL, "table would hold more elements than buckets (no slot to insert into)");
  if (is_wide(t)) {
    KwSlots nw;
    kh_status st = fresh_slots(t, new_cap, nw);
    return st != KH_OK ? st : relayout<Wide>(t, nw, ck, cv, noff, ncnt, PB, drop_marked, nullptr);
  }
  KhSlots nw;
  kh_status st = fresh_slots(t, new_cap, nw);
  if (st != KH_OK) return st;
  const bool from_empty = t->lsize == 0;
  if (!pre && !g_disable_fused_rebuild && new_cap >= 2 * (uint64_t)KH_L && total_after <= threshold(new_cap, 0.9f) &&
      (!noff || PB >= log2u(new_cap >> KH_LB)) &&
      (from_empty ? noff != nullptr
                  : (t->cur.cap >= 2 * (uint64_t)KH_L && (new_cap == t->cur.cap || new_cap == 2 * t->cur.cap)))) {
    const size_t keep_blk = t->blk, keep_off = t->off;
    KhFusedParams F;
    memset(&F, 0, sizeof(F));
    F.PB = PB; F.mode = KH_DEDUP_FIRST;
    F.R.Old = narrow(t->cur); F.R.drop_marked = drop_marked ? 1 : 0; F.R.ck = ck; F.R.cv = cv; F.R.noff = noff; F.R.ncnt = ncnt; F.R.PB = PB;
    if (from_empty) F.R.Old.cap = 0;
    FusedRun run;
    { kh_status fs = launch_fused(t, 1, F, nw, log2u(new_cap >> KH_LB), "k_rebuild_fused", &run); if (fs != KH_OK) return fs; }
    const uint32_t* ff = reinterpret_cast<const uint32_t*>(reinterpret_cast<const char*>(t->hpin) + 64);
    bool bad = false;
    for (int i = 0; i < KH_NFLAGS; ++i) bad = bad || ff[i] != 0;
    if (!bad && t->hpin[0] == total_after) {
      adopt_slots(t, nw);
      return KH_OK;
    }
    if (getenv("KH_DEBUG_FUSED"))
      fprintf(stderr, "[kmerhash_amd] fused rebuild rejected: placed %llu expected %llu flags=%u %u %u %u %u\n", (unsigned long long)t->hpin[0],
              (unsigned long long)total_after, ff[0], ff[1], ff[2], ff[3], ff[4]);
    if (ff[KH_FLAG_PROBE_OVERFLOW] && !ff[KH_FLAG_FUSE_INVALID]) {
      retire_slots(t, nw);
      return fail(t, KH_ERR_PROBE_OVERFLOW, kProbeOverflowText);
    }
    t->blk = keep_blk; t->off = keep_off;
  }
  return relayout<Narrow>(t, nw, ck, cv, noff, ncnt, PB, drop_marked, pre);
}

inline uint64_t rh_rehash_capacity(uint64_t c, uint64_t size, float max_lf) {
  if (size > 0) {
    if (0 >= threshold(c, max_lf)) c <<= 1;
    while (size > threshold(c, max_lf)) c <<= 1;
  }
  return c;
}
kh_status refuse_streaming(kh_table* t) { return fail(t, KH_ERR_INVALID, "a streamed insert is in progress (kh_insert_end first)"); }
kh_status do_rehash(kh_table* t, uint64_t b) {
  if (t->ins.active) return refuse_streaming(t);
  uint64_t n = next_pow2(b);
  if (n == t->cur.cap) return KH_OK;
  if (t->kind == KHK_RH) {
    n = rh_rehash_capacity(n, t->lsize, t->max_lf);
    if (n == t->cur.cap) return KH_OK;
  } else if (t->lsize > n) {
    return fail(t, KH_ERR_FULL, "ERROR: did not find any place to insert.  should not have happend (hashmap_linearprobe.hpp:408)");
  }
  { kh_status ps = arena_prepare(t, ws_rebuild(n)); if (ps != KH_OK) return ps; }
  return rebuild(t, n, nullptr, nullptr, nullptr, nullptr, 0, false, t->lsize);
}
kh_status do_reserve(kh_table* t, uint64_t n) {
  if (n > t->max_load) return do_rehash(t, static_cast<uint64_t>(static_cast<float>(n) / t->max_lf));
  return KH_OK;
}

struct Partitioned {
  ulonglong2* rec;
  uint64_t* part_off;
  uint32_t PB, nparts;
  ulonglong2* spare;
  uint64_t slot;
  const unsigned long long* cursor;
  uint32_t* overflow;
  int rec12;
};
const bool g_disable_slack = getenv("KH_DISABLE_SLACK_PARTITION") != nullptr;
const int g_xcd_swizzle = getenv("KH_DISABLE_XCD_SWIZZLE") ? 0 : 1;
const int g_xcd_fronts = getenv("KH_DISABLE_XCD_FRONTS") ? 0 : 1;
inline uint32_t xcd_fronts_min_tiles() { const char* e = getenv("KH_XCD_FRONTS_MIN_TILES"); return e ? (uint32_t)std::max(0, atoi(e)) : 4u; }
inline uint64_t part_buffer_records(uint64_t n, uint32_t PB, bool allow_slack, double vf = 1.0) {
  if (!allow_slack || g_disable_slack || PB <= 11 || n < (uint64_t(256) << PB)) return n;
  return (slack_slot((double)n / (double)(uint64_t(1) << PB), vf) << PB) + KH_PART_TILE;
}

kh_status partition_batch(kh_table* t, const char* kbase, uint32_t kstride, const char* vbase, uint32_t vstride,
                          uint32_t vconst, uint64_t n, uint64_t idx_base, uint32_t PB, ulonglong2* tmp, ulonglong2* fin, Partitioned& out,
                          bool allow_slack = false, int rec12 = 0, const SlackShared* shared = nullptr, bool force_slack = false, double vf = 1.0) {
  const uint32_t nparts = 1u << PB;
  out.slot = 0; out.cursor = nullptr; out.overflow = nullptr; out.rec12 = 0;
  if (shared || force_slack || part_buffer_records(n, PB, allow_slack, vf) != n) {
    const uint32_t B1 = (PB + 1) / 2, B2 = PB - B1, nb1 = 1u << B1, nb2 = 1u << B2;
    const uint64_t slot = shared ? shared->slot : slack_slot((double)n / (double)nparts, vf);
    const uint64_t slot1 = shared ? slack_slot((double)n / (double)nb1) : slot * nb2;
    uint32_t tps_sub = 0;
    const uint64_t sub_slot = (g_xcd_fronts && !shared) ? xcd_sub_slot(n, nb1, nb2, slot1, vf, KH_PART_TILE, xcd_fronts_min_tiles(), &tps_sub) : 0;
    unsigned long long *cur1, *cur2; uint64_t* starts; uint32_t* ovf;
    TAKE(cur1, unsigned long long, sub_slot ? (size_t)nb1 * 8 : nb1);
    if (shared) { cur2 = shared->cur2; starts = shared->starts; ovf = shared->ovf; }
    else { TAKE(cur2, unsigned long long, nparts); TAKE(starts, uint64_t, (size_t)nparts + 1); TAKE(ovf, uint32_t, 1); }
    const double mean1 = (double)n / (double)nb1;
    const uint64_t fill_cap = std::min<uint64_t>(slot1, (uint64_t)(mean1 + 9.0 * std::sqrt(mean1 * vf) + 16.0));
    const uint32_t tps = sub_slot ? tps_sub : (uint32_t)((fill_cap + KH_PART_TILE - 1) / KH_PART_TILE);
    const uint32_t max_tiles = (sub_slot ? nb1 * 8u : nb1) * tps;
    if (shared) hipLaunchKernelGGL(k_init_cursors, dim3((nb1 + 255) / 256), dim3(256), 0, t->stream, cur1, (uint64_t*)nullptr, (uint64_t)nb1, slot1);
    else hipLaunchKernelGGL(k_init_cursors2, dim3((nparts + 256) / 256), dim3(256), 0, t->stream, cur1, (uint64_t)nb1, slot1, sub_slot ? 8u : 1u, cur2, starts, (uint64_t)nparts, slot, ovf);
    KhPartParams P;
    memset(&P, 0, sizeof(P));
    P.idx_base = idx_base;
    P.xcd_swizzle = g_xcd_swizzle;
    P.kbase = kbase; P.kstride = kstride; P.vbase = vbase; P.vstride = vstride; P.vconst = vconst; P.n = n;
    P.ntiles = (uint32_t)((n + KH_PART_TILE - 1) / KH_PART_TILE);
    P.seed = t->seed; P.PB = PB; P.shift = B2; P.nb = nb1; P.cursor = cur1; P.orec = tmp; P.slot = slot1; P.overflow = ovf; P.dump = slot1 * nb1;
    P.sub_slot = sub_slot;
    { Launch L(t, "k_part_scatter");
      if (rec12 == 1) { KH_SWITCH_HASH(t->hash, hipLaunchKernelGGL((k_part_scatter<HASH, 1>), dim3(P.ntiles), dim3(KH_PART_THREADS), ((nb1 + 1u) & ~1u) * 8 + nb1 * 8, t->stream, P)); }
      else if (rec12 == 2) { KH_SWITCH_HASH(t->hash, hipLaunchKernelGGL((k_part_scatter<HASH, 2>), dim3(P.ntiles), dim3(KH_PART_THREADS), ((nb1 + 1u) & ~1u) * 8 + nb1 * 8, t->stream, P)); }
      else { KH_SWITCH_HASH(t->hash, hipLaunchKernelGGL((k_part_scatter<HASH, 0>), dim3(P.ntiles), dim3(KH_PART_THREADS), ((nb1 + 1u) & ~1u) * 8 + nb1 * 8, t->stream, P)); } }
    KhPartParams Q = P;
    Q.kbase = nullptr; Q.kstride = 0; Q.vbase = nullptr; Q.vstride = 0; Q.rec_in = tmp;
    Q.tiles = nullptr; Q.ntiles_dev = nullptr; Q.ntiles = max_tiles; Q.slot_in = sub_slot ? sub_slot : slot1; Q.cur_in = cur1; Q.tps = tps;
    Q.sub_slot = 0; Q.seg_shift = sub_slot ? 3u : 0u; Q.xcd_buckets = sub_slot ? 1 : 0;
    Q.shift = 0; Q.nb = nb2; Q.cursor = cur2; Q.orec = fin; Q.slot = slot; Q.dump = slot * nparts;
    { Launch L(t, "k_part_scatter");
      if (rec12 == 1) { KH_SWITCH_HASH(t->hash, hipLaunchKernelGGL((k_part_scatter<HASH, 1>), dim3(max_tiles), dim3(KH_PART_THREADS), ((nb2 + 1u) & ~1u) * 8 + nb2 * 8, t->stream, Q)); }
      else if (rec12 == 2) { KH_SWITCH_HASH(t->hash, hipLaunchKernelGGL((k_part_scatter<HASH, 2>), dim3(max_tiles), dim3(KH_PART_THREADS), ((nb2 + 1u) & ~1u) * 8 + nb2 * 8, t->stream, Q)); }
      else { KH_SWITCH_HASH(t->hash, hipLaunchKernelGGL((k_part_scatter<HASH, 0>), dim3(max_tiles), dim3(KH_PART_THREADS), ((nb2 + 1u) & ~1u) * 8 + nb2 * 8, t->stream, Q)); } }
    HIPCHK(hipGetLastError());
    out.rec = fin; out.part_off = starts; out.PB = PB; out.nparts = nparts; out.spare = tmp;
    out.slot = slot; out.cursor = cur2; out.overflow = ovf; out.rec12 = rec12;
    return KH_OK;
  }
  if (rec12 == 1) return fail(t, KH_ERR_HIP, "internal: record kind not available with exact offsets");
  ulonglong2* ar = nullptr; ulonglong2* br = fin;
  const uint32_t B1 = PB <= 11 ? PB : (PB + 1) / 2, B2 = PB - B1;
  const uint32_t nb1 = 1u << B1, nb2 = 1u << B2;
  ar = B2 ? tmp : fin;
  uint32_t* counts1; uint64_t* off1; unsigned long long* cur1;
  TAKE(counts1, uint32_t, nb1); TAKE(off1, uint64_t, nb1 + 1); TAKE(cur1, unsigned long long, nb1);
  KhPartParams P;
  memset(&P, 0, sizeof(P));
  P.idx_base = idx_base;
  P.xcd_swizzle = g_xcd_swizzle;
  P.kbase = kbase; P.kstride = kstride; P.vbase = vbase; P.vstride = vstride; P.vconst = vconst; P.rec_in = nullptr; P.n = n;
  P.tiles = nullptr; P.ntiles_dev = nullptr; P.ntiles = (uint32_t)((n + KH_PART_TILE - 1) / KH_PART_TILE);
  P.seed = t->seed; P.PB = PB; P.shift = B2; P.nb = nb1; P.counts = counts1; P.cursor = cur1;
  P.orec = ar;
  KhTile* tiles = nullptr; uint32_t* ntiles_dev = nullptr; uint32_t* counts2 = nullptr; uint64_t* off2 = nullptr; unsigned long long* cur2 = nullptr;
  const uint32_t max_tiles = (uint32_t)(n / KH_PART_TILE) + nb1 + 1;
  if (B2 > 0) {
    TAKE(tiles, KhTile, max_tiles); TAKE(ntiles_dev, uint32_t, 1);
    TAKE(counts2, uint32_t, nparts); TAKE(off2, uint64_t, nparts + 1); TAKE(cur2, unsigned long long, nparts);
    HIPCHK(hipMemsetAsync(counts2, 0, sizeof(uint32_t) * nparts, t->stream));
  }
  const bool full_hist = B2 > 0 && PB <= 18;
  if (full_hist) {
    const int ncu = cu_count(t);
    const uint32_t grid = (uint32_t)std::max<uint64_t>(1, std::min<uint64_t>((uint64_t)ncu, (n + 4095) / 4096));
    const uint32_t slice_bits = PB > 16 ? PB - 16 : 0;
    { Launch L(t, "k_part_hist");
      const size_t smem = (size_t)((nparts >> slice_bits) / 2) * 4;
      KH_SWITCH_HASH(t->hash,
                     if (smem > 65536) HIPCHK(hipFuncSetAttribute(reinterpret_cast<const void*>(&k_part_hist_full<HASH>),
                                                                  hipFuncAttributeMaxDynamicSharedMemorySize, (int)smem));
                     for (uint32_t sl = 0; sl < (1u << slice_bits); ++sl)
                       hipLaunchKernelGGL((k_part_hist_full<HASH>), dim3(grid), dim3(KH_FULLHIST_THREADS), smem, t->stream,
                                          kbase, kstride, n, t->seed, PB, sl, slice_bits, counts2)); }
    { Launch L(t, "k_scan");
      hipLaunchKernelGGL(k_scan_u32_to_u64, dim3(1), dim3(KH_SCAN_THREADS), 0, t->stream, counts2, (uint64_t)nparts, off2); }
    hipLaunchKernelGGL(k_seg_offsets, dim3((nb1 + 256) / 256), dim3(256), 0, t->stream, off2, nb1, nb2, off1, cur1);
  } else {
    HIPCHK(hipMemsetAsync(counts1, 0, sizeof(uint32_t) * nb1, t->stream));
    const uint32_t hist_grid = std::min<uint32_t>(P.ntiles, 1024);
    { Launch L(t, "k_part_hist");
      KH_SWITCH_HASH(t->hash, hipLaunchKernelGGL((k_part_hist<HASH>), dim3(hist_grid), dim3(KH_PART_THREADS), nb1 * 4, t->stream, P)); }
    { Launch L(t, "k_scan");
      hipLaunchKernelGGL(k_scan_u32_to_u64, dim3(1), dim3(KH_SCAN_THREADS), 0, t->stream, counts1, (uint64_t)nb1, off1); }
    HIPCHK(hipMemcpyAsync(cur1, off1, sizeof(uint64_t) * nb1, hipMemcpyDeviceToDevice, t->stream));
  }
  { Launch L(t, "k_part_scatter");
    if (rec12 == 2) { KH_SWITCH_HASH(t->hash, hipLaunchKernelGGL((k_part_scatter<HASH, 2>), dim3(P.ntiles), dim3(KH_PART_THREADS), ((nb1 + 1u) & ~1u) * 8 + nb1 * 8, t->stream, P)); }
    else { KH_SWITCH_HASH(t->hash, hipLaunchKernelGGL((k_part_scatter<HASH, 0>), dim3(P.ntiles), dim3(KH_PART_THREADS), ((nb1 + 1u) & ~1u) * 8 + nb1 * 8, t->stream, P)); } }
  out.rec12 = rec12 == 2 ? 2 : 0;
  if (B2 == 0) {
    out.rec = ar; out.part_off = off1; out.PB = PB; out.nparts = nparts;
    out.spare = tmp;
    HIPCHK(hipGetLastError());
    return KH_OK;
  }
  { Launch L(t, "k_make_tiles");
    hipLaunchKernelGGL(k_make_tiles, dim3(1), dim3(1024), 0, t->stream, off1, nb1, tiles, ntiles_dev); }
  KhPartParams Q = P;
  Q.kbase = nullptr; Q.kstride = 0;
  Q.vbase = nullptr; Q.vstride = 0; Q.rec_in = ar;
  Q.tiles = tiles; Q.ntiles_dev = ntiles_dev; Q.ntiles = max_tiles;
  Q.shift = 0; Q.nb = nb2; Q.counts = counts2; Q.cursor = cur2; Q.orec = br;
  if (!full_hist) {
    { Launch L(t, "k_part_hist");
      if (rec12 == 2) { KH_SWITCH_HASH(t->hash, hipLaunchKernelGGL((k_part_hist<HASH, true>), dim3(std::min<uint32_t>(max_tiles, 1024)), dim3(KH_PART_THREADS), nb2 * 4, t->stream, Q)); }
      else { KH_SWITCH_HASH(t->hash, hipLaunchKernelGGL((k_part_hist<HASH>), dim3(std::min<uint32_t>(max_tiles, 1024)), dim3(KH_PART_THREADS), nb2 * 4, t->stream, Q)); } }
    { Launch L(t, "k_scan");
      hipLaunchKernelGGL(k_scan_u32_to_u64, dim3(1), dim3(KH_SCAN_THREADS), 0, t->stream, counts2, (uint64_t)nparts, off2); }
  }
  HIPCHK(hipMemcpyAsync(cur2, off2, sizeof(uint64_t) * nparts, hipMemcpyDeviceToDevice, t->stream));
  { Launch L(t, "k_part_scatter");
    if (rec12 == 2) { KH_SWITCH_HASH(t->hash, hipLaunchKernelGGL((k_part_scatter<HASH, 2>), dim3(max_tiles), dim3(KH_PART_THREADS), ((nb2 + 1u) & ~1u) * 8 + nb2 * 8, t->stream, Q)); }
    else { KH_SWITCH_HASH(t->hash, hipLaunchKernelGGL((k_part_scatter<HASH, 0>), dim3(max_tiles), dim3(KH_PART_THREADS), ((nb2 + 1u) & ~1u) * 8 + nb2 * 8, t->stream, Q)); } }
  HIPCHK(hipGetLastError());
  out.rec = br; out.part_off = off2; out.PB = PB; out.nparts = nparts;
  out.spare = tmp;
  return KH_OK;
}

uint64_t capacity_after(const kh_table* t, uint64_t cap, uint64_t lsize, uint64_t ncalls, uint64_t dnew, uint64_t last_first) {
  if (ncalls == 0) return cap;
  uint64_t c = cap;
  if (lsize >= threshold(c, t->max_lf)) c <<= 1;
  const uint64_t fin = lsize + dnew;
  while (fin > threshold(c, t->max_lf)) c <<= 1;
  if (dnew > 0 && fin == threshold(c, t->max_lf) && last_first + 1 < ncalls) c <<= 1;
  return c;
}

enum { INS_FIRST = 0, INS_UPDATE = 1, INS_PLUS = 2, INS_MIN = 3, INS_MAX = 4, INS_OR = 5 };
inline bool is_reduce(int mode) { return mode >= INS_PLUS; }
inline int reduce_op(int mode) { return is_reduce(mode) ? mode - INS_PLUS : 0; }
inline bool one_launch_mode(int mode) { return mode == INS_FIRST || mode == INS_UPDATE || mode == INS_PLUS; }
inline const char* apply_label(int mode) { return mode == INS_PLUS ? "k_apply_plus" : "k_apply_reduce"; }
static_assert(KH_REDUCE_MIN == KH_ROP_MIN && KH_REDUCE_MAX == KH_ROP_MAX && KH_REDUCE_OR == KH_ROP_OR && KH_REDUCE_PLUS == KH_ROP_PLUS, "kh_reduce_op is the kernels' rop");
inline bool ins_flags_ok(unsigned flags) {
  if (flags & ~(unsigned)(KH_INS_REDUCE_PLUS | KH_INS_REPEATABLE | KH_INS_REDUCE_OP_MASK)) return false;
  return (flags & KH_INS_REDUCE_PLUS) || !(flags & KH_INS_REDUCE_OP_MASK);
}
inline int ins_flags_mode(unsigned flags) {
  return (flags & KH_INS_REDUCE_PLUS) ? INS_PLUS + (int)((flags & KH_INS_REDUCE_OP_MASK) >> KH_INS_REDUCE_OP_SHIFT) : INS_FIRST;
}
const uint64_t g_max_pass = getenv("KH_MAX_PASS_RECORDS") ? std::max<uint64_t>(1024, std::min<uint64_t>(strtoull(getenv("KH_MAX_PASS_RECORDS"), nullptr, 10), 0xFFFFFFF0ull))
                                                          : (uint64_t(1) << 30);
bool g_disable_fused = getenv("KH_DISABLE_FUSED_BUILD") != nullptr;

const kh_status KH_RETRY_EXACT = static_cast<kh_status>(100);
kh_status insert_finish(kh_table* t, KhSrcSet S, uint64_t n, uint32_t PB, uint64_t cap_u, int mode, uint64_t forced_cap,
                        ulonglong2* spare, uint64_t* n_new_out, uint64_t list_cap = 0);

inline bool fused_build_applies(const kh_table* t, uint64_t cap_u, uint32_t PB) {
  return t->lsize == 0 && cap_u >= 2 * (uint64_t)KH_L && t->max_lf <= 0.9f && PB == log2u(cap_u >> KH_LB) && !g_disable_fused;
}
inline bool nodup_build_applies(const kh_table* t, uint64_t cap_u, uint32_t PB, int mode) {
  return fused_build_applies(t, cap_u, PB) && t->batch_nodup && (mode == INS_FIRST || mode == INS_PLUS) && !getenv("KH_DISABLE_NODUP");
}

kh_status insert_core(kh_table* t, const char* kbase, uint32_t kstride, const char* vbase, uint32_t vstride,
                      uint64_t n, int mode, uint64_t forced_cap, uint64_t* n_new_out) {
  *n_new_out = 0;
  if (n == 0) return KH_OK;
  const uint64_t cap_u = forced_cap ? forced_cap : capacity_after(t, t->cur.cap, t->lsize, n, n, n - 1);
  const uint32_t PB = cap_u > KH_L ? log2u(cap_u >> KH_LB) : 0u;
  if (PB > 22) return fail(t, KH_ERR_UNSUPPORTED, "batch would need more than 2^22 partitions");
  const size_t keep_blk = t->blk, keep_off = t->off;
  int first_attempt = 0;
  bool dup_heavy = false;
  double vf = 1.0;
  if (part_buffer_records(n, PB, true) != n) {
    unsigned long long* sset; uint32_t* dups;
    TAKE(sset, unsigned long long, KH_SAMPLE_SET); TAKE(dups, uint32_t, 1);
    HIPCHK(hipMemsetAsync(sset, 0, sizeof(unsigned long long) * KH_SAMPLE_SET, t->stream));
    HIPCHK(hipMemsetAsync(dups, 0, 4, t->stream));
    { Launch L(t, "k_sample_dups");
      hipLaunchKernelGGL(k_sample_dups, dim3(KH_SAMPLE_N / 256), dim3(256), 0, t->stream, kbase, kstride, n, sset, dups); }
    HIPCHK(hipMemcpyAsync(t->hpin + 31, dups, 4, hipMemcpyDeviceToHost, t->stream));
    HIPCHK(hipStreamSynchronize(t->stream));
    const uint32_t dsample = (uint32_t)t->hpin[31];
    if (dsample >= 1u) {
      dup_heavy = true;
      const double d_ub = (double)dsample + 3.0 * std::sqrt((double)dsample) + 3.0;
      const double f = 1.0 + 2.0 * (double)n * d_ub / ((double)KH_SAMPLE_N * (double)KH_SAMPLE_N);
      const double mean = (double)n / (double)(uint64_t(1) << PB);
      if (!getenv("KH_DISABLE_DUP_SLACK") && (double)slack_slot(mean, f) <= 2.0 * mean) vf = f;
      else first_attempt = 1;
    }
    t->batch_nodup = dsample == 0u;
    t->blk = keep_blk; t->off = keep_off;
  } else first_attempt = 1;
  for (int attempt = first_attempt; attempt < 2; ++attempt) {
    const bool slack = attempt == 0;
    const uint64_t m = part_buffer_records(n, PB, slack, vf);
    if (!slack && attempt == 1) { t->blk = keep_blk; t->off = keep_off; }
    const bool rec12 = slack && t->batch_nodup && nodup_build_applies(t, cap_u, PB, mode);
    const bool rec8 = !rec12 && dup_heavy && mode == INS_PLUS && vbase == nullptr && !getenv("KH_DISABLE_REC8");
    const int kind = rec12 ? 1 : rec8 ? 2 : 0;
    ulonglong2 *tmp, *fin, *spare;
    { char *a, *b; const size_t rb = kind == 1 ? sizeof(KhRec12) : kind == 2 ? sizeof(KhRec8) : sizeof(ulonglong2);
      TAKE(a, char, m * rb); TAKE(b, char, m * rb);
      tmp = reinterpret_cast<ulonglong2*>(a); fin = reinterpret_cast<ulonglong2*>(b); spare = tmp;
      if (kind == 2) { char* c; TAKE(c, char, m * 12); spare = reinterpret_cast<ulonglong2*>(c); } }
    Partitioned R;
    kh_status st = partition_batch(t, kbase, kstride, vbase, vstride, mode == INS_PLUS ? 1u : 0u, n, 0, PB, tmp, fin, R, slack, kind, nullptr, false, vf);
    if (st != KH_OK) return st;
    KhSrcSet S;
    memset(&S, 0, sizeof(S));
    S.rec[0] = R.rec; S.off[0] = R.part_off; S.n = 1; S.merged_off = R.part_off; S.slot[0] = R.slot; S.cur[0] = R.cursor;
    S.rec12 = (uint32_t)R.rec12;
    t->part_overflow = R.overflow; t->batch_vf = vf;
    st = insert_finish(t, S, n, PB, cap_u, mode, forced_cap, spare, n_new_out, m);
    t->part_overflow = nullptr; t->batch_nodup = false; t->batch_vf = 1.0;
    if (st != KH_RETRY_EXACT) return st;
  }
  return fail(t, KH_ERR_HIP, "internal: exact partition reported a slot overflow");
}

kh_status insert_finish(kh_table* t, KhSrcSet S, uint64_t n, uint32_t PB, uint64_t cap_u, int mode, uint64_t forced_cap,
                        ulonglong2* spare, uint64_t* n_new_out, uint64_t list_cap) {
  *n_new_out = 0;
  if (list_cap < n) list_cap = n;
  kh_status st = KH_OK;
  const uint32_t nparts = 1u << PB;
  struct { uint32_t nparts; } R; R.nparts = nparts;
  if (fused_build_applies(t, cap_u, PB) && one_launch_mode(mode) && S.rec12 != 2 && !(t->batch_vf >= 2.0)) {
    const uint32_t nch = (uint32_t)(cap_u >> KH_LB);
    KhSlots nw;
    st = fresh_slots(t, cap_u, nw);
    if (st != KH_OK) return st;
    KhFusedParams F;
    memset(&F, 0, sizeof(F));
    F.src = S; F.PB = PB;
    F.mode = mode == INS_PLUS ? KH_DEDUP_PLUS : KH_DEDUP_FIRST;
    F.base_size = 0;
    F.n_total = n;
    F.nodup = nodup_build_applies(t, cap_u, PB, mode) ? 1 : 0;
    F.half_max_load = (cap_u >> 1) >= t->cur.cap ? threshold(cap_u >> 1, t->max_lf) : 0;
    FusedRun run;
    { kh_status fs = launch_fused(t, 0, F, nw, PB, "k_build_fused", &run); if (fs != KH_OK) return fs; }
    if (t->part_overflow && (uint32_t)t->hpin[30]) { retire_slots(t, nw); return KH_RETRY_EXACT; }
    unsigned long long* totals = run.totals;
    const uint64_t fd = t->hpin[0];
    const uint64_t flast = (mode == INS_PLUS || S.rec12) ? n - 1 : (t->hpin[1] ? t->hpin[1] - 1 : 0);
    const uint32_t* ff = reinterpret_cast<const uint32_t*>(reinterpret_cast<const char*>(t->hpin) + 64);
    bool bad = S.rec12 && fd != n;
    for (int i = 0; i < KH_NFLAGS; ++i) bad = bad || ff[i] != 0;
    if (!bad && capacity_after(t, t->cur.cap, t->lsize, n, fd, flast) == cap_u) {
      adopt_slots(t, nw);
      t->lsize = fd;
      *n_new_out = fd;
      if (mode == INS_UPDATE) {
        KhDedupParams A;
        memset(&A, 0, sizeof(A));
        A.src = S; A.T = narrow(t->cur); A.seed = t->seed; A.table_empty = 0; A.mode = KH_DEDUP_LAST;
        uint32_t* cn; TAKE(cn, uint32_t, R.nparts);
        A.cnt_new = cn; A.max_idx_plus1 = totals; A.flags = F.flags; A.count_cap = 0; A.PB = PB;
        Launch L(t, "k_dedup_assign");
        KH_SWITCH_KIND_HASH(t->kind, t->hash, hipLaunchKernelGGL((k_dedup<KIND, HASH>), dim3(R.nparts), dim3(KH_CHUNK_THREADS), 0, t->stream, A));
        HIPCHK(hipGetLastError());
      }
      return KH_OK;
    }
    if (getenv("KH_DEBUG_FUSED"))
      fprintf(stderr, "[kmerhash_amd] fused build rejected: n=%llu dnew=%llu cap_u=%llu cap_rule=%llu flags=%u %u %u %u %u est=%u/%u/%u\n", (unsigned long long)n,
              (unsigned long long)fd, (unsigned long long)cap_u, (unsigned long long)capacity_after(t, t->cur.cap, t->lsize, n, fd, flast), ff[0], ff[1], ff[2], ff[3], ff[4],
              reinterpret_cast<const uint32_t*>(reinterpret_cast<const char*>(t->hpin) + 32)[1], reinterpret_cast<const uint32_t*>(reinterpret_cast<const char*>(t->hpin) + 32)[0],
              reinterpret_cast<const uint32_t*>(reinterpret_cast<const char*>(t->hpin) + 32)[2]);
    retire_slots(t, nw);
    if (S.rec12 == 1) return KH_RETRY_EXACT;
  }
  if (S.rec12 == 1) return fail(t, KH_ERR_HIP, "internal: 12-byte records outside the bulk build");
  if (t->lsize > 0 && S.rec12 != 2 && (mode == INS_FIRST || mode == INS_PLUS) && !forced_cap && !g_disable_fused_rebuild &&
      t->cur.cap >= 2 * (uint64_t)KH_L && (cap_u == t->cur.cap || cap_u == 2 * t->cur.cap) && t->max_lf <= 0.9f &&
      PB == log2u(cap_u >> KH_LB) && t->lsize + n <= threshold(cap_u, 0.92f)) {
    const size_t keep_blk = t->blk, keep_off = t->off;
    const uint32_t nch = (uint32_t)(cap_u >> KH_LB);
    KhSlots nw;
    st = fresh_slots(t, cap_u, nw);
    if (st != KH_OK) return st;
    KhFusedParams F;
    memset(&F, 0, sizeof(F));
    F.src = S; F.PB = PB;
    F.mode = mode == INS_PLUS ? KH_DEDUP_PLUS : KH_DEDUP_FIRST;
    F.n_total = n;
    F.base_size = t->lsize;
    F.half_max_load = (cap_u >> 1) >= t->cur.cap ? threshold(cap_u >> 1, t->max_lf) : 0;
    F.R.Old = narrow(t->cur); F.R.PB = PB;
    FusedRun run;
    const bool ordered = t->kind == KHK_RH && cap_u == t->cur.cap && S.n == 1 && S.rec12 == 0 &&
                         (S.slot[0] ? S.slot[0] <= KH_IS_MAXR : n / (uint64_t(1) << PB) <= KH_IS_MAXR / 2) && !getenv("KH_DISABLE_ORDERED_INSERT");
    { kh_status fs = launch_fused(t, ordered ? 5 : 2, F, nw, PB, "k_insert_fused", &run); if (fs != KH_OK) return fs; }
    if (t->part_overflow && (uint32_t)t->hpin[30]) { retire_slots(t, nw); return KH_RETRY_EXACT; }
    const uint64_t total = t->hpin[0];
    const uint64_t fd = total >= t->lsize ? total - t->lsize : 0;
    const uint64_t flast = mode == INS_PLUS ? n - 1 : (t->hpin[1] ? t->hpin[1] - 1 : 0);
    const uint32_t* ff = reinterpret_cast<const uint32_t*>(reinterpret_cast<const char*>(t->hpin) + 64);
    bool bad = total < t->lsize;
    for (int i = 0; i < KH_NFLAGS; ++i) bad = bad || ff[i] != 0;
    if (!bad && capacity_after(t, t->cur.cap, t->lsize, n, fd, flast) == cap_u) {
      adopt_slots(t, nw);
      t->lsize = total;
      *n_new_out = fd;
      return KH_OK;
    }
    if (getenv("KH_DEBUG_FUSED"))
      fprintf(stderr, "[kmerhash_amd] fused insert rejected: n=%llu size=%llu total=%llu cap_u=%llu cap_rule=%llu flags=%u %u %u %u %u\n", (unsigned long long)n,
              (unsigned long long)t->lsize, (unsigned long long)total, (unsigned long long)cap_u,
              (unsigned long long)capacity_after(t, t->cur.cap, t->lsize, n, fd, flast), ff[0], ff[1], ff[2], ff[3], ff[4]);
    retire_slots(t, nw);
    t->blk = keep_blk; t->off = keep_off;
  }
  uint32_t* cnt_new; uint64_t* noff; unsigned long long* scal; uint32_t* flags;
  TAKE(cnt_new, uint32_t, R.nparts); TAKE(noff, uint64_t, R.nparts + 1); TAKE(scal, unsigned long long, 4);
  TAKE(flags, uint32_t, KH_NFLAGS);
  HIPCHK(hipMemsetAsync(scal, 0, sizeof(unsigned long long) * 4, t->stream));
  HIPCHK(hipMemsetAsync(flags, 0, sizeof(uint32_t) * KH_NFLAGS, t->stream));
  KhDedupParams D;
  D.src = S;
  D.nk = reinterpret_cast<uint64_t*>(spare); D.nv = reinterpret_cast<uint32_t*>(reinterpret_cast<char*>(spare) + list_cap * 8);
  D.cnt_new = cnt_new; D.max_idx_plus1 = scal;
  PreCount pre; pre.homecnt = nullptr; pre.sumA = nullptr; pre.sumN = nullptr;
  const bool fuse = t->lsize == 0;
// ... 595 lines not shown
  if (mx) *mx = t->max_lf;
  if (cur) *cur = static_cast<float>(t->lsize) / static_cast<float>(t->cur.cap);
  return KH_OK;
}
kh_status kh_clear(kh_table* t) {
  if (!t) return KH_ERR_INVALID;
  if (t->ins.active) return refuse_streaming(t);
  HIPCHK(hipSetDevice(t->device));
  t->lsize = 0;
  { kh_status fs = fill_empty(t, t->cur); if (fs != KH_OK) return fs; }
  HIPCHK(hipStreamSynchronize(t->stream));
  return KH_OK;
}
kh_status kh_reserve(kh_table* t, uint64_t n) { if (!t) return KH_ERR_INVALID; HIPCHK(hipSetDevice(t->device)); return do_reserve(t, n); }
kh_status kh_rehash(kh_table* t, uint64_t b) { if (!t) return KH_ERR_INVALID; HIPCHK(hipSetDevice(t->device)); return do_rehash(t, b); }

kh_status kh_insert(kh_table* t, const void* keys, const void* vals, uint64_t n, kh_mem where, uint64_t* n_inserted) {
  if (!t) return KH_ERR_INVALID;
  return do_insert(t, keys, 8, vals, 4, n, where, INS_FIRST, n_inserted);
}
kh_status kh_insert_pairs(kh_table* t, const void* pairs16, uint64_t n, kh_mem where, uint64_t* n_inserted) {
  if (!t) return KH_ERR_INVALID;
  return do_insert(t, pairs16, 16, pairs16 ? static_cast<const char*>(pairs16) + 8 : nullptr, 16, n, where, INS_FIRST, n_inserted);
}
kh_status kh_insert_one(kh_table* t, uint64_t key, uint32_t val, uint64_t* n_inserted) {
  if (!t) return KH_ERR_INVALID;
  return do_insert(t, &key, 8, &val, 4, 1, KH_MEM_HOST, INS_FIRST, n_inserted, false);
}
kh_status kh_update(kh_table* t, const void* keys, const void* vals, uint64_t n, kh_mem where, uint64_t* n_inserted) {
  if (!t) return KH_ERR_INVALID;
  return do_insert(t, keys, 8, vals, 4, n, where, INS_UPDATE, n_inserted);
}
kh_status kh_insert_begin(kh_table* t, uint64_t n_total, int reduce_plus) {
  return kh_insert_begin_ex(t, n_total, reduce_plus ? KH_INS_REDUCE_PLUS : 0u);
}
kh_status kh_insert_begin_ex(kh_table* t, uint64_t n_total, unsigned flags) {
  if (!t) return KH_ERR_INVALID;
  if (t->ins.active) return fail(t, KH_ERR_INVALID, "a streamed insert is already in progress");
  if (!ins_flags_ok(flags)) return fail(t, KH_ERR_INVALID, "unknown flag");
  HIPCHK(hipSetDevice(t->device));
  memset(&t->ins, 0, sizeof(t->ins));
  t->ins.mode = ins_flags_mode(flags);
  t->ins.repeatable = (flags & KH_INS_REPEATABLE) != 0 && !g_disable_slack;
  t->ins.n_total = n_total;
  const uint64_t cu = capacity_after(t, t->cur.cap, t->lsize, n_total ? n_total : 1, n_total, n_total ? n_total - 1 : 0);
  { kh_status ps = arena_prepare(t, n_total * ((flags & KH_INS_REPEATABLE) ? 72 : 56) + ws_rebuild(cu) + cu * 2 + (cu > KH_L ? (cu >> KH_LB) : 1) * 64 * (KH_MAX_SRC + 1) +
                                    (n_total / KH_PART_TILE + 4096 * KH_MAX_SRC) * 16 + (size_t(8) << 20));
    if (ps != KH_OK) return ps; }
  const uint32_t PB = cu > KH_L ? log2u(cu >> KH_LB) : 0u;
  t->ins.fallback = n_total == 0 || n_total > 0xFFFFFFF0ull || PB > 22 || t->lsize >= threshold(t->cur.cap << 1, t->max_lf);
  t->ins.cap_u = cu; t->ins.PB = PB;
  if (n_total) {
    if (t->ins.fallback) { TAKE(t->ins.stage_k, uint64_t, n_total); TAKE(t->ins.stage_v, uint32_t, n_total); }
    else if (!t->ins.repeatable) { TAKE(t->ins.tmp, ulonglong2, n_total); TAKE(t->ins.fin, ulonglong2, n_total); }
  }
  t->ins.active = true;
  return KH_OK;
}

kh_status kh_insert_feed(kh_table* t, const void* keys, const void* vals, uint64_t n, kh_mem where) {
  if (!t) return KH_ERR_INVALID;
  if (!t->ins.active) return fail(t, KH_ERR_INVALID, "kh_insert_feed without kh_insert_begin");
  if (n == 0) return KH_OK;
  if (!keys) return fail(t, KH_ERR_INVALID, "null keys");
  if (!vals && is_reduce(t->ins.mode) && t->ins.mode != INS_PLUS) return fail(t, KH_ERR_INVALID, "null values: only the std::plus reducer has a default value (1)");
  if (t->ins.fed + n > t->ins.n_total) return fail(t, KH_ERR_INVALID, "more pairs fed than announced to kh_insert_begin");
  HIPCHK(hipSetDevice(t->device));
  const uint64_t* dk; const uint32_t* dv;
  kh_status st = stage_in<uint64_t>(t, keys, n, where, &dk);
  if (st == KH_OK) st = stage_in<uint32_t>(t, vals, n, where, &dv);
  if (st != KH_OK) return st;
  if (t->ins.fallback) {
    HIPCHK(hipMemcpyAsync(t->ins.stage_k + t->ins.fed, dk, n * 8, hipMemcpyDeviceToDevice, t->stream));
    if (dv) HIPCHK(hipMemcpyAsync(t->ins.stage_v + t->ins.fed, dv, n * 4, hipMemcpyDeviceToDevice, t->stream));
    else HIPCHK(hipMemsetD32Async(reinterpret_cast<hipDeviceptr_t>(t->ins.stage_v + t->ins.fed), t->ins.mode == INS_PLUS ? 1 : 0, n, t->stream));
  } else {
    if (t->ins.S.n == KH_MAX_SRC) return fail(t, KH_ERR_UNSUPPORTED, "more than 16 feeds in one streamed insert");
    if (t->ins.S.n == 0 && n >= KH_SAMPLE_N) {
      unsigned long long* sset; uint32_t* dups;
      TAKE(sset, unsigned long long, KH_SAMPLE_SET); TAKE(dups, uint32_t, 1);
      HIPCHK(hipMemsetAsync(sset, 0, sizeof(unsigned long long) * KH_SAMPLE_SET, t->stream));
      HIPCHK(hipMemsetAsync(dups, 0, 4, t->stream));
      { Launch L(t, "k_sample_dups");
        hipLaunchKernelGGL(k_sample_dups, dim3(KH_SAMPLE_N / 256), dim3(256), 0, t->stream, reinterpret_cast<const char*>(dk), 8u, n, sset, dups); }
      HIPCHK(hipMemcpyAsync(t->hpin + 31, dups, 4, hipMemcpyDeviceToHost, t->stream));
      HIPCHK(hipStreamSynchronize(t->stream));
      t->ins.nodup = (uint32_t)t->hpin[31] == 0u;
      t->ins.slack = t->ins.repeatable && (uint32_t)t->hpin[31] == 0u && part_buffer_records(t->ins.n_total, t->ins.PB, true) != t->ins.n_total;
    }
    if (t->ins.S.n == 0 && t->ins.repeatable) {
      const uint64_t nt = t->ins.n_total;
      if (t->ins.slack) {
        const uint32_t nparts = 1u << t->ins.PB;
        t->batch_nodup = t->ins.nodup;
        t->ins.rec12 = nodup_build_applies(t, t->ins.cap_u, t->ins.PB, t->ins.mode);
        t->batch_nodup = false;
        SlackShared& sh = t->ins.sh;
        sh.slot = slack_slot((double)nt / (double)nparts);
        char* f; TAKE(f, char, (sh.slot * nparts + KH_PART_TILE) * (t->ins.rec12 ? sizeof(KhRec12) : sizeof(ulonglong2)));
        t->ins.fin = reinterpret_cast<ulonglong2*>(f);
        TAKE(sh.cur2, unsigned long long, nparts); TAKE(sh.starts, uint64_t, (size_t)nparts + 1); TAKE(sh.ovf, uint32_t, 1);
        HIPCHK(hipMemsetAsync(sh.ovf, 0, 4, t->stream));
        hipLaunchKernelGGL(k_init_cursors, dim3((nparts + 256) / 256), dim3(256), 0, t->stream, sh.cur2, sh.starts, (uint64_t)nparts, sh.slot);
      } else { TAKE(t->ins.tmp, ulonglong2, nt); TAKE(t->ins.fin, ulonglong2, nt); }
    }
    Partitioned R;
    if (t->ins.slack) {
      const uint32_t B1 = (t->ins.PB + 1) / 2, nb1 = 1u << B1;
      const uint64_t slot1 = slack_slot((double)n / (double)nb1);
      char* tm; TAKE(tm, char, (slot1 * nb1 + KH_PART_TILE) * (t->ins.rec12 ? sizeof(KhRec12) : sizeof(ulonglong2)));
      st = partition_batch(t, reinterpret_cast<const char*>(dk), 8, reinterpret_cast<const char*>(dv), 4, t->ins.mode == INS_PLUS ? 1u : 0u,
                           n, t->ins.fed, t->ins.PB, reinterpret_cast<ulonglong2*>(tm), t->ins.fin, R, true, t->ins.rec12, &t->ins.sh);
      if (st != KH_OK) return st;
      t->ins.S.n = 1;
    } else {
      st = partition_batch(t, reinterpret_cast<const char*>(dk), 8, reinterpret_cast<const char*>(dv), 4, t->ins.mode == INS_PLUS ? 1u : 0u,
                           n, t->ins.fed, t->ins.PB, t->ins.tmp, t->ins.fin + t->ins.fed, R);
      if (st != KH_OK) return st;
      t->ins.S.rec[t->ins.S.n] = R.rec; t->ins.S.off[t->ins.S.n] = R.part_off; ++t->ins.S.n;
    }
  }
  t->ins.fed += n;
  if (where == KH_MEM_HOST) HIPCHK(hipStreamSynchronize(t->stream));
  return KH_OK;
}

kh_status kh_insert_end(kh_table* t, uint64_t* n_inserted) {
  if (n_inserted) *n_inserted = 0;
  if (!t) return KH_ERR_INVALID;
  if (!t->ins.active) return fail(t, KH_ERR_INVALID, "kh_insert_end without kh_insert_begin");
  t->ins.active = false;
  if (t->ins.fed != t->ins.n_total) return fail(t, KH_ERR_INVALID, "fewer pairs fed than announced to kh_insert_begin");
  HIPCHK(hipSetDevice(t->device));
  uint64_t nn = 0;
  kh_status st = KH_OK;
  const uint64_t n = t->ins.n_total;
  if (n) {
    if (t->ins.fallback) {
      st = insert_device(t, reinterpret_cast<const char*>(t->ins.stage_k), 8, reinterpret_cast<const char*>(t->ins.stage_v), 4, n, t->ins.mode, &nn);
    } else if (t->ins.slack) {
      const uint32_t nparts = 1u << t->ins.PB;
      const uint64_t list_cap = t->ins.sh.slot * nparts + KH_PART_TILE;
      KhSrcSet S;
      memset(&S, 0, sizeof(S));
      S.rec[0] = t->ins.fin; S.off[0] = t->ins.sh.starts; S.n = 1; S.merged_off = t->ins.sh.starts;
      S.slot[0] = t->ins.sh.slot; S.cur[0] = t->ins.sh.cur2; S.rec12 = t->ins.rec12 ? 1u : 0u;
      char* spare; TAKE(spare, char, list_cap * 16);
      t->part_overflow = t->ins.sh.ovf; t->batch_nodup = t->ins.nodup;
      st = insert_finish(t, S, n, t->ins.PB, t->ins.cap_u, t->ins.mode, 0, reinterpret_cast<ulonglong2*>(spare), &nn, list_cap);
      t->part_overflow = nullptr; t->batch_nodup = false;
      if (st == KH_RETRY_EXACT) {
        if (n_inserted) *n_inserted = 0;
        HIPCHK(hipStreamSynchronize(t->stream));
        t->err = "the speculative partition of this repeatable streamed insert did not hold: feed the same pieces again (kh_insert_begin without KH_INS_REPEATABLE)";
        return KH_ERR_RETRY;
      }
    } else {
      KhSrcSet S = t->ins.S;
      if (S.n == 1) S.merged_off = S.off[0];
      else {
        uint64_t* mo;
        const uint64_t nq1 = (uint64_t(1) << t->ins.PB) + 1;
        TAKE(mo, uint64_t, nq1);
        hipLaunchKernelGGL(k_merge_offsets, dim3((uint32_t)((nq1 + 255) / 256)), dim3(256), 0, t->stream, S, nq1, mo);
        S.merged_off = mo;
      }
      t->batch_nodup = t->ins.nodup;
// ... 2161 lines not shown
```

Measured before the change: 47.64 billion.

## Run duplicate sampling optimistically on device and fuse tail launches

Removes the host synchronization after duplicate sampling by assuming no duplicates. The sample now runs fused with cursor initialization, and the partition and fused build kernels early-exit via a device-side skip flag. When the sample finds duplicates, the host detects it after the build and retries with the old path. The tail kernels are merged: carry computation, the lean-path totals reduction (via striped atomic counters) and the tail chunk placement now run in one kernel, and the overflow and dup status come back in the existing pinned copy. This trades extra wasted work and a retry on duplicate-heavy inputs for fewer launches and syncs on the common path.

```diff
diff --git a/kmerhash_amd/csrc/kh_kernels.h b/kmerhash_amd/csrc/kh_kernels.h
--- a/kmerhash_amd/csrc/kh_kernels.h
+++ b/kmerhash_amd/csrc/kh_kernels.h
@@ -512,6 +512,7 @@
   int xcd_swizzle;
   uint64_t slot_in; const unsigned long long* cur_in; uint32_t tps;
   uint64_t sub_slot; uint32_t seg_shift; int xcd_buckets;
+  const uint32_t* skip;
 };
 
 __device__ __forceinline__ uint32_t kh_part_q(uint64_t h, uint32_t PB) {
@@ -603,6 +604,7 @@
   const uint32_t tid = threadIdx.x, lane = tid & 63, wid = tid >> 6;
   const uint32_t ntiles = P.tiles ? *P.ntiles_dev : P.ntiles;
   if (blockIdx.x >= ntiles) return;
+  if (P.skip && *P.skip) return;
   uint32_t tile = blockIdx.x;
   const uint32_t xcd = blockIdx.x & 7u;
   if (P.xcd_buckets) {
@@ -818,9 +820,24 @@
 
 #define KH_SAMPLE_N 65536u
 #define KH_SAMPLE_SET (1u << 18)
+struct KhCursorInit {
+  unsigned long long* cur1; uint64_t n1, slot1; uint32_t sub1;
+  unsigned long long* cur2; uint64_t* starts; uint64_t n2, slot2;
+  uint32_t* ovf;
+};
+__device__ __forceinline__ void kh_init_cursors2(const KhCursorInit& I, uint64_t i) {
+  if (i < I.n1 * I.sub1) I.cur1[i] = (i / I.sub1) * I.slot1 + (i % I.sub1) * (I.slot1 / I.sub1);
+  if (i < I.n2) I.cur2[i] = i * I.slot2;
+  if (i <= I.n2) I.starts[i] = i * I.slot2;
+  if (i == 0) *I.ovf = 0u;
+}
 __global__ void k_sample_dups(const char* __restrict__ kbase, uint32_t kstride, uint64_t n, unsigned long long* __restrict__ set ,
-                              uint32_t* __restrict__ dups) {
+                              uint32_t* __restrict__ dups, KhCursorInit I) {
   const uint32_t i = blockIdx.x * blockDim.x + threadIdx.x;
+  if (I.cur2) {
+    const uint64_t words = I.n1 * I.sub1 > I.n2 + 1 ? I.n1 * I.sub1 : I.n2 + 1;
+    for (uint64_t w = i; w < words; w += (uint64_t)gridDim.x * blockDim.x) kh_init_cursors2(I, w);
+  }
   if (i >= KH_SAMPLE_N) return;
   const uint64_t pos = (uint64_t)i * (n / KH_SAMPLE_N);
   const unsigned long long key = *reinterpret_cast<const uint64_t*>(kbase + pos * kstride) ^ 0x8000000000000001ull;
@@ -834,14 +851,7 @@
   }
 }
 
-__global__ void k_init_cursors2(unsigned long long* __restrict__ cur1, uint64_t n1, uint64_t slot1, uint32_t sub1, unsigned long long* __restrict__ cur2,
-                                uint64_t* __restrict__ starts, uint64_t n2, uint64_t slot2, uint32_t* __restrict__ ovf) {
-  const uint64_t i = (uint64_t)blockIdx.x * blockDim.x + threadIdx.x;
-  if (i < n1 * sub1) cur1[i] = (i / sub1) * slot1 + (i % sub1) * (slot1 / sub1);
-  if (i < n2) cur2[i] = i * slot2;
-  if (i <= n2) starts[i] = i * slot2;
-  if (i == 0) *ovf = 0u;
-}
+__global__ void k_init_cursors2(KhCursorInit I) { kh_init_cursors2(I, (uint64_t)blockIdx.x * blockDim.x + threadIdx.x); }
 __global__ void k_init_cursors(unsigned long long* __restrict__ cursor, uint64_t* __restrict__ starts, uint64_t n, uint64_t slot) {
   const uint64_t i = (uint64_t)blockIdx.x * blockDim.x + threadIdx.x;
   if (i < n) cursor[i] = i * slot;
@@ -1539,8 +1549,8 @@
 }
 
 #define KH_SPILL 256
-template <int KIND, int HASH>
-__global__ __launch_bounds__(KH_CHUNK_THREADS) void k_chunk_place(KhRebuildParams P) {
+template <int KIND, int HASH, bool TAIL>
+__device__ __forceinline__ void kh_chunk_place(const KhRebuildParams& P, const uint32_t c, const long long xcarry, const uint32_t n0) {
   __shared__ uint64_t skeys[KH_L + KH_SPILL];
   __shared__ uint32_t svals[KH_L + KH_SPILL];
   __shared__ uint32_t sinfo_w[(KH_L + KH_SPILL) / 4];
@@ -1550,7 +1560,7 @@
   __shared__ long long s_pend;
   __shared__ KhMP s_wtot[KH_CHUNK_THREADS / 64];
   uint8_t* sinfo = reinterpret_cast<uint8_t*>(sinfo_w);
-  const uint32_t tid = threadIdx.x, c = blockIdx.x;
+  const uint32_t tid = threadIdx.x;
   const uint32_t Ln = P.New.cap > KH_L ? KH_L : (uint32_t)P.New.cap;
   const uint64_t Sc = (uint64_t)c * Ln, mask_n = P.New.cap - 1;
   const uint32_t empty4 = KIND == KHK_RH ? 0u : 0x40404040u;
@@ -1566,7 +1576,7 @@
     fill[tid * KH_HOMES_PER_THREAD + j] = 0;
   }
   KhMP excl = kh_block_scan_mp(v, s_wtot, nullptr);
-  const long long xr = P.xcarry[c] - (long long)Sc;
+  const long long xr = xcarry - (long long)Sc;
   long long p = excl.A > xr + excl.n ? excl.A : xr + excl.n;
 #pragma unroll
   for (uint32_t j = 0; j < KH_HOMES_PER_THREAD; ++j) {
@@ -1593,7 +1603,9 @@
     else kh_slot_st(P.New.s + ((Sc + prel) & mask_n), key, val, ib);
   };
   kh_for_each_old<KIND, HASH>(P, c, &s_emin, place);
-  kh_for_each_new<HASH>(P, c, place);
+  if (TAIL) {
+    for (uint32_t i = tid; i < n0; i += KH_CHUNK_THREADS) { const uint64_t key = P.ck[i]; place(key, P.cv[i], kh_hash64<HASH>(key, P.seed) & mask_n); }
+  } else kh_for_each_new<HASH>(P, c, place);
   __syncthreads();
   long long pend = s_pend;
   if (pend < (long long)Ln) pend = Ln;
@@ -1603,6 +1615,8 @@
     kh_slot_st(P.New.s + ((Sc + s0) & mask_n), skeys[s0], svals[s0], sinfo[s0]);
   }
 }
+template <int KIND, int HASH>
+__global__ __launch_bounds__(KH_CHUNK_THREADS) void k_chunk_place(KhRebuildParams P) { kh_chunk_place<KIND, HASH, false>(P, blockIdx.x, P.xcarry[blockIdx.x], 0u); }
 
 #define KH_XB 127u
 #define KH_FSPILL 128u
@@ -1619,7 +1633,11 @@
   long long poll_limit;
   int nodup;
   KhRebuildParams R;
+  const uint32_t* skip;
+  unsigned long long* cnt;
 };
+#define KH_FUSED_NCNT 64u
+#define KH_FUSED_CNT_STRIDE 16u
 
 template <int KIND, int HASH, bool MERGE>
 __device__ __forceinline__ uint32_t kh_stage_from_table(const KhRebuildParams& R, uint32_t c, uint64_t Sc, unsigned long long* lk,
@@ -1736,6 +1754,7 @@
   const uint64_t cap = P.New.cap, mask_n = cap - 1;
   const uint32_t nch = (uint32_t)(cap >> KH_LB);
   KH_STAMP(0);
+  if (SRC == 0 && P.skip && *P.skip) return;
   if (tid == 0) {
     s_chunk = blockIdx.x;
     s_max = 0;
@@ -2136,6 +2155,7 @@
   const uint64_t Sc = (uint64_t)c * KH_L;
   const unsigned long long VALID = 1ull << 63;
   KH_STAMP_L(0);
+  if (P.skip && *P.skip) return;
   if (tid == 0) s_abort = (uint32_t)__hip_atomic_load(&P.est[1], __ATOMIC_RELAXED, __HIP_MEMORY_SCOPE_AGENT);
   const uint32_t q = P.PB ? (__brev(c) >> (32 - P.PB)) : 0u;
   const KhRec12* src; uint32_t m;
@@ -2211,7 +2231,7 @@
     if (tid == 0) {
       if (!early) atomicOr(&P.flags[KH_FLAG_FUSE_INVALID], 1u);
       __hip_atomic_store(&P.pub[0], VALID | ((unsigned long long)spill0 << 32) | n_c, __ATOMIC_RELAXED, __HIP_MEMORY_SCOPE_AGENT);
-      P.maxidx[0] = 0;
+      (void)__hip_atomic_fetch_add(&P.cnt[0], (unsigned long long)n_c, __ATOMIC_RELAXED, __HIP_MEMORY_SCOPE_AGENT);
     }
 #pragma unroll
     for (uint32_t j = 0; j < KH_HOMES_PER_THREAD; ++j) P.homecnt0[tid * KH_HOMES_PER_THREAD + j] = (uint16_t)cb[j];
@@ -2220,6 +2240,7 @@
   }
   unsigned long long w0 = 0;
   if (tid == 0) {
+    (void)__hip_atomic_fetch_add(&P.cnt[(c & (KH_FUSED_NCNT - 1u)) * KH_FUSED_CNT_STRIDE], (unsigned long long)n_c, __ATOMIC_RELAXED, __HIP_MEMORY_SCOPE_AGENT);
     if (c < 64) {
       const unsigned long long mine = ((unsigned long long)n_c << 32) | m;
       const unsigned long long tot = atomicAdd(&P.est[0], mine) + mine;
@@ -2234,7 +2255,6 @@
     }
     if (early) __hip_atomic_store(&P.pub[c], VALID | ((unsigned long long)spill0 << 32) | n_c, __ATOMIC_RELAXED, __HIP_MEMORY_SCOPE_AGENT);
     w0 = __hip_atomic_load(&P.pub[c - 1], __ATOMIC_RELAXED, __HIP_MEMORY_SCOPE_AGENT);
-    P.maxidx[c] = 0;
   }
   {
     long long p = excl.A > (long long)excl.n ? excl.A : excl.n;
@@ -2903,13 +2923,24 @@
   (void)n_old;
 }
 
-__global__ void k_fused_tail_carry(const unsigned long long* __restrict__ pub, uint32_t nch, long long* __restrict__ xcarry0,
-                                   uint64_t* __restrict__ noff0 = nullptr, uint32_t* __restrict__ ncnt0 = nullptr) {
-  if (threadIdx.x == 0 && blockIdx.x == 0) {
-    xcarry0[0] = (long long)((pub[nch - 1] >> 32) & 0x7FFFFFFFull);
-    if (noff0) { noff0[0] = 0; noff0[1] = 0; }
-    if (ncnt0) ncnt0[0] = (uint32_t)pub[0];
-  }
+struct KhTailParams {
+  const unsigned long long* pub; uint32_t nch;
+  const unsigned long long* cnt; unsigned long long* totals;
+  const uint32_t* skip; const uint32_t* ovf; uint32_t* status;
+};
+template <int KIND, int HASH>
+__global__ __launch_bounds__(KH_CHUNK_THREADS) void k_fused_tail(KhRebuildParams P, KhTailParams E) {
+  const uint32_t dups = E.skip ? *E.skip : 0u;
+  if (threadIdx.x == 0) { E.status[0] = dups; E.status[1] = E.ovf ? *E.ovf : 0u; }
+  if (dups) return;
+  if (E.cnt && threadIdx.x < 64) {
+    static_assert(KH_FUSED_NCNT == 64, "one count word per lane of the first wave");
+    unsigned long long sum = E.cnt[threadIdx.x * KH_FUSED_CNT_STRIDE];
+    for (int off = 32; off > 0; off >>= 1) sum += __shfl_down(sum, off, 64);
+    if (threadIdx.x == 0) E.totals[0] = sum;
+  }
+  const long long xcarry = (long long)((E.pub[E.nch - 1] >> 32) & 0x7FFFFFFFull);
+  kh_chunk_place<KIND, HASH, true>(P, 0u, xcarry, (uint32_t)E.pub[0]);
 }
 
 __global__ __launch_bounds__(1024) void k_fused_totals(const unsigned long long* __restrict__ pub, const uint32_t* __restrict__ maxidx, uint32_t nch,
diff --git a/kmerhash_amd/csrc/kmerhash_amd.hip b/kmerhash_amd/csrc/kmerhash_amd.hip
--- a/kmerhash_amd/csrc/kmerhash_amd.hip
+++ b/kmerhash_amd/csrc/kmerhash_amd.hip
@@ -150,6 +150,8 @@
   uint32_t* part_overflow = nullptr;
   double batch_vf = 1.0;
   bool batch_nodup = false;
+  uint32_t* sample_dups = nullptr;
+  char* fused_blk = nullptr; size_t fused_blk_bytes = 0;
   bool prof = false;
   std::vector<ProfRec> recs;
   std::vector<std::pair<std::string, std::pair<double, uint64_t> > > prof_acc;
@@ -451,49 +453,57 @@
 const long long g_poll_limit = getenv("KH_DEBUG_POLL_LIMIT") ? atoll(getenv("KH_DEBUG_POLL_LIMIT")) : (1ll << 23);
 struct FusedRun { unsigned long long* totals; uint32_t* flags; };
 const bool g_disable_lean = getenv("KH_DISABLE_LEAN_BUILD") != nullptr;
+inline size_t fused_blk_bytes(uint32_t nch) { return (size_t)nch * 12 + 256 + (size_t)KH_FUSED_NCNT * KH_FUSED_CNT_STRIDE * 8; }
 kh_status launch_fused(kh_table* t, int src, KhFusedParams& F, const KhSlots& nw, uint32_t PB_tail, const char* name, FusedRun* out) {
   const uint32_t nch = (uint32_t)(nw.cap >> KH_LB);
-  char* blk; uint32_t* maxidx; uint64_t* ck0; uint32_t* cv0; uint16_t* hc0; long long* xc0; uint64_t* noff0; uint32_t* ncnt0;
-  const size_t sz_pub = (size_t)nch * 8, sz_ctl = sz_pub + 256, sz_all = sz_ctl + (size_t)nch * 4;
-  TAKE(blk, char, sz_all);
+  char* blk; uint32_t* maxidx; uint64_t* ck0; uint32_t* cv0; uint16_t* hc0;
+  const size_t sz_pub = (size_t)nch * 8, sz_ctl = sz_pub + 256, sz_all = fused_blk_bytes(nch);
+  if (t->fused_blk && t->fused_blk_bytes == sz_all) blk = t->fused_blk;
+  else { TAKE(blk, char, sz_all); HIPCHK(hipMemsetAsync(blk, 0, sz_all, t->stream)); }
+  t->fused_blk = nullptr;
   maxidx = reinterpret_cast<uint32_t*>(blk + sz_ctl);
-  TAKE(ck0, uint64_t, KH_DD_M); TAKE(cv0, uint32_t, KH_DD_M); TAKE(hc0, uint16_t, KH_L); TAKE(xc0, long long, 1);
-  TAKE(noff0, uint64_t, 2); TAKE(ncnt0, uint32_t, 1);
-  HIPCHK(hipMemsetAsync(blk, 0, sz_all, t->stream));
+  TAKE(ck0, uint64_t, KH_DD_M); TAKE(cv0, uint32_t, KH_DD_M); TAKE(hc0, uint16_t, KH_L);
   F.New = nw; F.seed = t->seed;
   F.pub = reinterpret_cast<unsigned long long*>(blk);
   unsigned long long* totals = reinterpret_cast<unsigned long long*>(blk + sz_pub);
   F.maxidx = maxidx; F.ck0 = ck0; F.cv0 = cv0; F.homecnt0 = hc0;
+  F.cnt = reinterpret_cast<unsigned long long*>(blk + sz_ctl + (size_t)nch * 4);
+  F.skip = src == 0 ? t->sample_dups : nullptr;
   F.est = reinterpret_cast<unsigned long long*>(blk + sz_pub + 32);
   F.flags = reinterpret_cast<uint32_t*>(blk + sz_pub + 64);
   F.poll_limit = g_poll_limit;
   F.R.New = nw; F.R.seed = t->seed; F.R.flags = F.flags;
+  bool lean = false;
   { Launch L(t, name);
     const double mean_c = (double)F.n_total / (double)nch;
     const bool lean_fits = mean_c + 5.0 * std::sqrt(mean_c) < (double)KH_LEAN_M;
-    if (src == 0 && F.nodup && F.src.rec12 == 1 && F.src.n == 1 && lean_fits && !g_disable_lean) { KH_SWITCH_KIND_HASH(t->kind, t->hash, hipLaunchKernelGGL((k_build_lean<KIND, HASH>), dim3(nch), dim3(KH_CHUNK_THREADS), 0, t->stream, F)); }
+    lean = src == 0 && F.nodup && F.src.rec12 == 1 && F.src.n == 1 && lean_fits && !g_disable_lean;
+    if (lean) { KH_SWITCH_KIND_HASH(t->kind, t->hash, hipLaunchKernelGGL((k_build_lean<KIND, HASH>), dim3(nch), dim3(KH_CHUNK_THREADS), 0, t->stream, F)); }
     else if (src == 0) { KH_SWITCH_KIND_HASH(t->kind, t->hash, hipLaunchKernelGGL((k_build_fused<KIND, HASH, 0>), dim3(nch), dim3(KH_CHUNK_THREADS), 0, t->stream, F)); }
     else if (src == 1) { KH_SWITCH_KIND_HASH(t->kind, t->hash, hipLaunchKernelGGL((k_build_fused<KIND, HASH, 1>), dim3(nch), dim3(KH_CHUNK_THREADS), 0, t->stream, F)); }
     else if (src == 3) { KH_SWITCH_HASH(t->hash, hipLaunchKernelGGL((k_build_fused<KHK_RH, HASH, 3>), dim3(nch), dim3(KH_CHUNK_THREADS), 0, t->stream, F)); }
     else if (src == 4) { KH_SWITCH_HASH(t->hash, hipLaunchKernelGGL((k_erase_stream<HASH>), dim3(nch), dim3(KH_CHUNK_THREADS), 0, t->stream, F)); }
     else if (src == 5) { KH_SWITCH_HASH(t->hash, hipLaunchKernelGGL((k_insert_stream<HASH>), dim3(nch), dim3(KH_CHUNK_THREADS), 0, t->stream, F)); }
     else { KH_SWITCH_KIND_HASH(t->kind, t->hash, hipLaunchKernelGGL((k_build_fused<KIND, HASH, 2>), dim3(nch), dim3(KH_CHUNK_THREADS), 0, t->stream, F)); } }
-  { Launch L(t, "k_fused_totals");
+  if (!lean) { Launch L(t, "k_fused_totals");
     hipLaunchKernelGGL(k_fused_totals, dim3(std::max<uint32_t>(1u, std::min<uint32_t>(64u, nch / 1024u))), dim3(1024), 0, t->stream, F.pub, maxidx, nch, totals); }
   {
     Launch L(t, "k_fused_tail");
-    hipLaunchKernelGGL(k_fused_tail_carry, dim3(1), dim3(64), 0, t->stream, F.pub, nch, xc0, noff0, ncnt0);
     KhRebuildParams T0;
     memset(&T0, 0, sizeof(T0));
-    T0.Old = kNoSlots; T0.New = nw; T0.ck = ck0; T0.cv = cv0; T0.noff = noff0; T0.ncnt = ncnt0; T0.PB = PB_tail;
-    T0.seed = t->seed; T0.homecnt = hc0; T0.xcarry = xc0; T0.flags = F.flags;
-    KH_SWITCH_KIND_HASH(t->kind, t->hash, hipLaunchKernelGGL((k_chunk_place<KIND, HASH>), dim3(1), dim3(KH_CHUNK_THREADS), 0, t->stream, T0));
+    T0.Old = kNoSlots; T0.New = nw; T0.ck = ck0; T0.cv = cv0; T0.PB = PB_tail;
+    T0.seed = t->seed; T0.homecnt = hc0; T0.flags = F.flags;
+    KhTailParams E;
+    E.pub = F.pub; E.nch = nch; E.cnt = lean ? F.cnt : nullptr; E.totals = totals;
+    E.skip = F.skip; E.ovf = t->part_overflow; E.status = reinterpret_cast<uint32_t*>(blk + sz_pub + 16);
+    KH_SWITCH_KIND_HASH(t->kind, t->hash, hipLaunchKernelGGL((k_fused_tail<KIND, HASH>), dim3(1), dim3(KH_CHUNK_THREADS), 0, t->stream, T0, E));
   }
   HIPCHK(hipGetLastError());
   HIPCHK(hipMemcpyAsync(t->hpin, blk + sz_pub, 128, hipMemcpyDeviceToHost, t->stream));
-  t->hpin[30] = 0;
-  if (t->part_overflow) HIPCHK(hipMemcpyAsync(t->hpin + 30, t->part_overflow, 4, hipMemcpyDeviceToHost, t->stream));
   HIPCHK(hipStreamSynchronize(t->stream));
+  { const uint32_t* status = reinterpret_cast<const uint32_t*>(t->hpin + 2);
+    t->hpin[31] = status[0];
+    t->hpin[30] = status[1]; }
   out->totals = totals; out->flags = F.flags;
   return KH_OK;
 }
@@ -652,9 +662,11 @@
   return (slack_slot((double)n / (double)(uint64_t(1) << PB), vf) << PB) + KH_PART_TILE;
 }
 
+struct SampleRun { unsigned long long* set; uint32_t* dups; };
 kh_status partition_batch(kh_table* t, const char* kbase, uint32_t kstride, const char* vbase, uint32_t vstride,
                           uint32_t vconst, uint64_t n, uint64_t idx_base, uint32_t PB, ulonglong2* tmp, ulonglong2* fin, Partitioned& out,
-                          bool allow_slack = false, int rec12 = 0, const SlackShared* shared = nullptr, bool force_slack = false, double vf = 1.0) {
+                          bool allow_slack = false, int rec12 = 0, const SlackShared* shared = nullptr, bool force_slack = false, double vf = 1.0,
+                          const SampleRun* sample = nullptr) {
   const uint32_t nparts = 1u << PB;
   out.slot = 0; out.cursor = nullptr; out.overflow = nullptr; out.rec12 = 0;
   if (shared || force_slack || part_buffer_records(n, PB, allow_slack, vf) != n) {
@@ -672,9 +684,16 @@
     const uint32_t tps = sub_slot ? tps_sub : (uint32_t)((fill_cap + KH_PART_TILE - 1) / KH_PART_TILE);
     const uint32_t max_tiles = (sub_slot ? nb1 * 8u : nb1) * tps;
     if (shared) hipLaunchKernelGGL(k_init_cursors, dim3((nb1 + 255) / 256), dim3(256), 0, t->stream, cur1, (uint64_t*)nullptr, (uint64_t)nb1, slot1);
-    else hipLaunchKernelGGL(k_init_cursors2, dim3((nparts + 256) / 256), dim3(256), 0, t->stream, cur1, (uint64_t)nb1, slot1, sub_slot ? 8u : 1u, cur2, starts, (uint64_t)nparts, slot, ovf);
+    else {
+      KhCursorInit I;
+      I.cur1 = cur1; I.n1 = nb1; I.slot1 = slot1; I.sub1 = sub_slot ? 8u : 1u; I.cur2 = cur2; I.starts = starts; I.n2 = nparts; I.slot2 = slot; I.ovf = ovf;
+      if (sample) { Launch L(t, "k_sample_dups");
+        hipLaunchKernelGGL(k_sample_dups, dim3(KH_SAMPLE_N / 256), dim3(256), 0, t->stream, kbase, kstride, n, sample->set, sample->dups, I); }
+      else hipLaunchKernelGGL(k_init_cursors2, dim3((nparts + 256) / 256), dim3(256), 0, t->stream, I);
+    }
     KhPartParams P;
     memset(&P, 0, sizeof(P));
+    P.skip = sample ? sample->dups : nullptr;
     P.idx_base = idx_base;
     P.xcd_swizzle = g_xcd_swizzle;
     P.kbase = kbase; P.kstride = kstride; P.vbase = vbase; P.vstride = vstride; P.vconst = vconst; P.n = n;
@@ -808,6 +827,8 @@
 bool g_disable_fused = getenv("KH_DISABLE_FUSED_BUILD") != nullptr;
 
 const kh_status KH_RETRY_EXACT = static_cast<kh_status>(100);
+const kh_status KH_RETRY_DUPS = static_cast<kh_status>(101);
+const bool g_sync_sample = getenv("KH_DISABLE_OPTIMISTIC_SAMPLE") != nullptr;
 kh_status insert_finish(kh_table* t, KhSrcSet S, uint64_t n, uint32_t PB, uint64_t cap_u, int mode, uint64_t forced_cap,
                         ulonglong2* spare, uint64_t* n_new_out, uint64_t list_cap = 0);
 
@@ -829,16 +850,7 @@
   int first_attempt = 0;
   bool dup_heavy = false;
   double vf = 1.0;
-  if (part_buffer_records(n, PB, true) != n) {
-    unsigned long long* sset; uint32_t* dups;
-    TAKE(sset, unsigned long long, KH_SAMPLE_SET); TAKE(dups, uint32_t, 1);
-    HIPCHK(hipMemsetAsync(sset, 0, sizeof(unsigned long long) * KH_SAMPLE_SET, t->stream));
-    HIPCHK(hipMemsetAsync(dups, 0, 4, t->stream));
-    { Launch L(t, "k_sample_dups");
-      hipLaunchKernelGGL(k_sample_dups, dim3(KH_SAMPLE_N / 256), dim3(256), 0, t->stream, kbase, kstride, n, sset, dups); }
-    HIPCHK(hipMemcpyAsync(t->hpin + 31, dups, 4, hipMemcpyDeviceToHost, t->stream));
-    HIPCHK(hipStreamSynchronize(t->stream));
-    const uint32_t dsample = (uint32_t)t->hpin[31];
+  auto decide = [&](uint32_t dsample) {
     if (dsample >= 1u) {
       dup_heavy = true;
       const double d_ub = (double)dsample + 3.0 * std::sqrt((double)dsample) + 3.0;
@@ -848,12 +860,35 @@
       else first_attempt = 1;
     }
     t->batch_nodup = dsample == 0u;
-    t->blk = keep_blk; t->off = keep_off;
-  } else first_attempt = 1;
+  };
+  const bool slackable = part_buffer_records(n, PB, true) != n;
+  bool optimistic = slackable && fused_build_applies(t, cap_u, PB) && one_launch_mode(mode) && !g_sync_sample;
+  if (slackable && !optimistic) {
+    unsigned long long* sset; uint32_t* dups;
+    { char* b; TAKE(b, char, sizeof(unsigned long long) * KH_SAMPLE_SET + 256);
+      sset = reinterpret_cast<unsigned long long*>(b); dups = reinterpret_cast<uint32_t*>(b + sizeof(unsigned long long) * KH_SAMPLE_SET);
+      HIPCHK(hipMemsetAsync(b, 0, sizeof(unsigned long long) * KH_SAMPLE_SET + 256, t->stream)); }
+    { Launch L(t, "k_sample_dups");
+      hipLaunchKernelGGL(k_sample_dups, dim3(KH_SAMPLE_N / 256), dim3(256), 0, t->stream, kbase, kstride, n, sset, dups, KhCursorInit{}); }
+    HIPCHK(hipMemcpyAsync(t->hpin + 31, dups, 4, hipMemcpyDeviceToHost, t->stream));
+    HIPCHK(hipStreamSynchronize(t->stream));
+    decide((uint32_t)t->hpin[31]);
+  } else if (!slackable) first_attempt = 1;
   for (int attempt = first_attempt; attempt < 2; ++attempt) {
     const bool slack = attempt == 0;
     const uint64_t m = part_buffer_records(n, PB, slack, vf);
-    if (!slack && attempt == 1) { t->blk = keep_blk; t->off = keep_off; }
+    t->blk = keep_blk; t->off = keep_off;
+    SampleRun sample;
+    const size_t rec0 = t->recs.size();
+    if (optimistic) {
+      const size_t fb = (fused_blk_bytes((uint32_t)(cap_u >> KH_LB)) + 255) & ~size_t(255), hb = fb + 256 + sizeof(unsigned long long) * KH_SAMPLE_SET;
+      char* head; TAKE(head, char, hb);
+      HIPCHK(hipMemsetAsync(head, 0, hb, t->stream));
+      t->fused_blk = head; t->fused_blk_bytes = fused_blk_bytes((uint32_t)(cap_u >> KH_LB));
+      sample.dups = reinterpret_cast<uint32_t*>(head + fb); sample.set = reinterpret_cast<unsigned long long*>(head + fb + 256);
+      t->sample_dups = sample.dups;
+      t->batch_nodup = true;
+    }
     const bool rec12 = slack && t->batch_nodup && nodup_build_applies(t, cap_u, PB, mode);
     const bool rec8 = !rec12 && dup_heavy && mode == INS_PLUS && vbase == nullptr && !getenv("KH_DISABLE_REC8");
     const int kind = rec12 ? 1 : rec8 ? 2 : 0;
@@ -863,15 +898,25 @@
       tmp = reinterpret_cast<ulonglong2*>(a); fin = reinterpret_cast<ulonglong2*>(b); spare = tmp;
       if (kind == 2) { char* c; TAKE(c, char, m * 12); spare = reinterpret_cast<ulonglong2*>(c); } }
     Partitioned R;
-    kh_status st = partition_batch(t, kbase, kstride, vbase, vstride, mode == INS_PLUS ? 1u : 0u, n, 0, PB, tmp, fin, R, slack, kind, nullptr, false, vf);
-    if (st != KH_OK) return st;
-    KhSrcSet S;
-    memset(&S, 0, sizeof(S));
-    S.rec[0] = R.rec; S.off[0] = R.part_off; S.n = 1; S.merged_off = R.part_off; S.slot[0] = R.slot; S.cur[0] = R.cursor;
-    S.rec12 = (uint32_t)R.rec12;
-    t->part_overflow = R.overflow; t->batch_vf = vf;
-    st = insert_finish(t, S, n, PB, cap_u, mode, forced_cap, spare, n_new_out, m);
-    t->part_overflow = nullptr; t->batch_nodup = false; t->batch_vf = 1.0;
+    kh_status st = partition_batch(t, kbase, kstride, vbase, vstride, mode == INS_PLUS ? 1u : 0u, n, 0, PB, tmp, fin, R, slack, kind, nullptr, false, vf,
+                                   optimistic ? &sample : nullptr);
+    if (st == KH_OK) {
+      KhSrcSet S;
+      memset(&S, 0, sizeof(S));
+      S.rec[0] = R.rec; S.off[0] = R.part_off; S.n = 1; S.merged_off = R.part_off; S.slot[0] = R.slot; S.cur[0] = R.cursor;
+      S.rec12 = (uint32_t)R.rec12;
+      t->part_overflow = R.overflow; t->batch_vf = vf;
+      st = insert_finish(t, S, n, PB, cap_u, mode, forced_cap, spare, n_new_out, m);
+    }
+    t->part_overflow = nullptr; t->batch_nodup = false; t->batch_vf = 1.0; t->sample_dups = nullptr; t->fused_blk = nullptr;
+    const bool was_optimistic = optimistic;
+    optimistic = false;
+    if (st == KH_RETRY_DUPS && was_optimistic) {
+      decide((uint32_t)t->hpin[31]);
+      for (size_t i = rec0; i < t->recs.size(); ++i) if (strcmp(t->recs[i].name, "k_sample_dups")) t->recs[i].name = "k_attempt_skipped";
+      attempt = first_attempt - 1;
+      continue;
+    }
     if (st != KH_RETRY_EXACT) return st;
   }
   return fail(t, KH_ERR_HIP, "internal: exact partition reported a slot overflow");
@@ -899,6 +944,7 @@
     F.half_max_load = (cap_u >> 1) >= t->cur.cap ? threshold(cap_u >> 1, t->max_lf) : 0;
     FusedRun run;
     { kh_status fs = launch_fused(t, 0, F, nw, PB, "k_build_fused", &run); if (fs != KH_OK) return fs; }
+    if (F.skip && (uint32_t)t->hpin[31]) { retire_slots(t, nw); return KH_RETRY_DUPS; }
     if (t->part_overflow && (uint32_t)t->hpin[30]) { retire_slots(t, nw); return KH_RETRY_EXACT; }
     unsigned long long* totals = run.totals;
     const uint64_t fd = t->hpin[0];
@@ -1660,7 +1706,7 @@
       HIPCHK(hipMemsetAsync(sset, 0, sizeof(unsigned long long) * KH_SAMPLE_SET, t->stream));
       HIPCHK(hipMemsetAsync(dups, 0, 4, t->stream));
       { Launch L(t, "k_sample_dups");
-        hipLaunchKernelGGL(k_sample_dups, dim3(KH_SAMPLE_N / 256), dim3(256), 0, t->stream, reinterpret_cast<const char*>(dk), 8u, n, sset, dups); }
+        hipLaunchKernelGGL(k_sample_dups, dim3(KH_SAMPLE_N / 256), dim3(256), 0, t->stream, reinterpret_cast<const char*>(dk), 8u, n, sset, dups, KhCursorInit{}); }
       HIPCHK(hipMemcpyAsync(t->hpin + 31, dups, 4, hipMemcpyDeviceToHost, t->stream));
       HIPCHK(hipStreamSynchronize(t->stream));
       t->ins.nodup = (uint32_t)t->hpin[31] == 0u;
```

After: 48.33 billion, median of 6. 1.01x the previous value.
